# stardist/stardist

Hardware: AMD Instinct MI355X
Metric: predict_instances() Mpix/s (2D) + Mvox/s (3D) end-to-end at 1/2/4/8 GPU (higher is better)
Workload: dtype f32

## Files before the change

### include/stardist_hip.h

```cpp
#ifndef STARDIST_HIP_H
#define STARDIST_HIP_H

#include <stdbool.h>
#include <stdint.h>

#ifdef __cplusplus
extern "C" {
#endif

const char* sd_last_error(void);
int sd_version(void);
int sd_device_count(void);
int sd_release_workspace(void);
int sd_set_option(const char* name, int value);
int sd_get_option(const char* name);

int sd_nms2d_host(const float* dist, const float* points, int n_polys, int n_rays,
                  int use_kdtree, int use_bbox, int verbose, float threshold,
                  uint8_t* keep, int64_t* stats);
int sd_nms2d_device(const float* d_dist, const float* d_points, int n_polys, int n_rays,
                    int use_kdtree, int use_bbox, int verbose, float threshold,
                    uint8_t* d_keep, int64_t* stats, void* stream);

int sd_nms2d_old_host(const int32_t* polys, int n_polys, int n_rays, const int32_t* mapping, int height, int width,
                      float threshold, int max_bbox_search, int grid_y, int grid_x, int verbose, uint8_t* keep);
int sd_nms2d_old_device(const int32_t* d_polys, int n_polys, int n_rays, const int32_t* d_mapping, int height, int width,
                        float threshold, int max_bbox_search, int grid_y, int grid_x, int verbose, uint8_t* d_keep, void* stream);

int sd_prepare_polys_device(const int32_t* d_x, const int32_t* d_y, int n_polys, int n_verts, void* d_out,
                            int64_t out_bytes, void* stream);

int sd_clip_pairs_device(const int32_t* d_xa, const int32_t* d_ya, const int32_t* d_xb,
                         const int32_t* d_yb, int n_pairs, int n_verts,
                         int64_t* d_out_twice_area, int32_t* d_out_flags, void* stream);

int sd_area_bounds_pairs_device(const int32_t* d_xa, const int32_t* d_ya, const int32_t* d_xb, const int32_t* d_yb, int n_pairs,
                                int n_verts, float* d_out_area, float* d_out_band, int32_t* d_out_info, void* stream);

int sd_poly_pass_device(const int32_t* d_x, const int32_t* d_y, int n_polys, int n_verts, void* d_props, void* d_prep, void* stream);

int sd_star_dist2d_host(const uint16_t* src, int H, int W, int n_rays, int grid_y, int grid_x,
                        float* dst);
int sd_star_dist2d_device(const uint16_t* d_src, int H, int W, int n_rays, int grid_y,
                          int grid_x, float* d_dst, void* stream);
int sd_star_dist3d_host(const uint16_t* src, int Z, int Y, int X, const float* dz,
                        const float* dy, const float* dx, int n_rays, int grid_z, int grid_y,
                        int grid_x, float* dst);
int sd_star_dist3d_device(const uint16_t* d_src, int Z, int Y, int X, const float* d_dz,
                          const float* d_dy, const float* d_dx, int n_rays, int grid_z,
                          int grid_y, int grid_x, float* d_dst, void* stream);

int sd_edt_prob_device(const int32_t* d_lbl, int Z, int Y, int X, double sz, double sy, double sx, int max_label,
                       float* d_prob, void* stream);

int sd_polygons_to_label_host(const float* coord, const int32_t* labels, int n_polys, int n_rays,
                              int H, int W, int32_t* result);
int sd_polygons_to_label_device(const float* d_coord, const int32_t* d_labels, int n_polys,
                                int n_rays, int H, int W, int32_t* d_result, void* stream);
int sd_polygons_to_label_window_device(const float* d_coord, const int32_t* d_labels, int n_polys, int n_rays, int HI, int WI,
                                       int y0, int x0, int H, int W, int32_t* d_result, void* stream);

int sd_dist_to_coord_device(const float* d_dist, const double* d_points, const double* d_sincos, long long n_polys, int n_rays,
                            double scale_y, double scale_x, float* d_coord, void* stream);

int sd_survivor_positions_device(const unsigned char* d_keep, long long n, long long* d_positions, int32_t* d_count, void* stream);
int sd_survivors2d_device(const long long* d_positions, int m, const float* d_prob, const long long* d_points, const float* d_dist,
                          int n_rays, const double* d_sincos, float* d_out_prob, long long* d_out_points, float* d_out_coord,
                          float* d_out_coord_paint, int32_t* d_out_labels_paint, void* stream);

void _LIB_non_maximum_suppression_sparse(const float* scores, const float* dist,
                                         const float* points, const int n_polys,
                                         const int n_rays, const int n_faces, const float* verts,
                                         const int* faces, const float threshold,
                                         const int use_bbox, const int use_kdtree,
                                         const int verbose, bool* result);
int sd_nms3d_device(const float* d_scores, const float* d_dist, const float* d_points,
                    int n_polys, int n_rays, int n_faces, const float* d_verts,
                    const int* d_faces, float threshold, int use_bbox, int use_kdtree,
                    int verbose, uint8_t* d_keep, int64_t* stats, void* stream);

int sd_hiv_pairs_device(const float* d_dist, const float* d_points, int n_polys, int n_rays, int n_faces,
                        const float* d_verts, const int* d_faces, const int32_t* d_pairs, int n_pairs,
                        double* d_vol_kernel, double* d_vol_hull, void* stream);

void _LIB_polyhedron_to_label(const float* dist, const float* points, const float* verts,
                              const int* faces, const int n_polys, const int n_rays,
                              const int n_faces, const int* labels, const int nz, const int ny,
                              const int nx, const int render_mode, const int verbose,
                              const int use_overlap_label, const int overlap_label, int* result);
int sd_polyhedron_to_label_device(const float* d_dist, const float* d_points,
                                  const float* d_verts, const int* d_faces, int n_polys,
                                  int n_rays, int n_faces, const int* d_labels, int nz, int ny,
                                  int nx, int render_mode, int verbose, int use_overlap_label,
                                  int overlap_label, int* d_result, void* stream);
int sd_polyhedron_to_label_window_device(const float* d_dist, const float* d_points, const float* d_verts, const int* d_faces,
                                         int n_polys, int n_rays, int n_faces, const int* d_labels, int NZ, int NY, int NX,
                                         int z0, int y0, int x0, int nz, int ny, int nx, int render_mode, int verbose,
                                         int use_overlap_label, int overlap_label, int* d_result, void* stream);

int sd_select_candidates_device(const float* d_prob, const float* d_dist, int ndim,
                                const int* shape, const int* b, int n_rays, float thresh,
                                int cap, float* d_out_prob, float* d_out_dist,
                                int32_t* d_out_points, int32_t* d_count, void* stream);

int sd_sort_scores_desc_device(const float* d_scores, int n, float* d_sorted, int64_t* d_order, void* stream);

int sd_sorted_rows_device(const int32_t* d_points, const int64_t* d_order, int n, int ndim, const int* full_shape, const int* origin,
                          const int* grid, int64_t* d_rows, float* d_points_f32, int64_t* d_points_i64, void* stream);

void _LIB_non_maximum_suppression_2d(const float* dist, const float* points, const int n_polys,
                                     const int n_rays, const float threshold, const int use_bbox,
                                     const int use_kdtree, const int verbose, bool* result);
void _LIB_polygon_to_label(const float* coord, const int* labels, const int n_polys,
                           const int n_rays, const int ny, const int nx, int* result);
void _LIB_star_dist(const unsigned short* src, const int ny, const int nx, const int n_rays,
                    const int grid_y, const int grid_x, float* dst);
void _LIB_star_dist3d(const unsigned short* src, const int nz, const int ny, const int nx,
                      const float* pdz, const float* pdy, const float* pdx, const int n_rays,
                      const int grid_z, const int grid_y, const int grid_x, float* dst);

int sd_bias_act_device(float* d_x, const float* d_bias, long long n_outer, int n_channels,
                       long long inner, int act, void* stream);
int sd_add_bias_act_device(float* d_x, const float* d_addend, const float* d_bias, long long n_outer,
                           int n_channels, long long inner, int act, void* stream);

int sd_maxpool_ndhwc_device(const float* d_in, int n_channels, int D, int H, int W, int pz, int py, int px, float* d_out, void* stream);

int sd_inside_polyhedron_device(const float* d_dist, const float* d_centre, int n_rays, int n_faces,
                                const float* d_verts, const int* d_faces, const float* d_points,
                                long long n, int use_cone_map, uint8_t* d_out, void* stream);

int sd_bias_act_dot_device(const float* d_in, float* d_out, const float* d_bias, long long n_pix, int n_channels,
                           int act, const float* d_w, const float* d_wbias, int sigmoid, float* d_dot, void* stream);
int sd_head_rows_device(const float* d_feat, int n_channels, const long long* d_rows, long long n_rows,
                        const float* d_w, const float* d_bias, int n_out, float clamp_min, float* d_out,
                        void* stream);

long long sd_conv3_packed_floats(int c_in, int c_out, int kz);
int sd_conv3_pack_weights_host(const float* w , int c_in, int c_out, int kz, float* packed);
int sd_conv3_ndhwc_device(const float* d_src0, int c0, int stride0, int up0, const float* d_src1, int c1, int stride1, int up1,
                          int D, int H, int W, int kz, const float* d_wpacked, const float* d_bias, int c_out, int act,
                          float* d_out, void* stream);
int sd_conv3_res_ndhwc_device(const float* d_src0, int c0, int stride0, int up0, const float* d_src1, int c1, int stride1, int up1,
                              int D, int H, int W, int kz, const float* d_wpacked, const float* d_bias, const float* d_res,
                              int res_stride, int c_out, int act, float* d_out, void* stream);

long long sd_conv3_bf16x6_packed_floats(int c_in, int c_out, int kz);
int sd_conv3_bf16x6_pack_weights_host(const float* w , int c_in, int c_out, int kz, float* packed);
int sd_conv3_bf16x6_ndhwc_device(const float* d_src0, int c0, int stride0, int up0, const float* d_src1, int c1, int stride1,
                                 int up1, int D, int H, int W, int kz, const float* d_wpacked, const float* d_bias, int c_out,
                                 int act, float* d_out, void* stream);
int sd_conv3_bf16x6_res_ndhwc_device(const float* d_src0, int c0, int stride0, int up0, const float* d_src1, int c1, int stride1,
                                     int up1, int D, int H, int W, int kz, const float* d_wpacked, const float* d_bias,
                                     const float* d_res, int res_stride, int c_out, int act, float* d_out, void* stream);

long long sd_conv3_f16x3_packed_floats(int c_in, int c_out, int kz);
int sd_conv3_f16x3_pack_weights_host(const float* w , int c_in, int c_out, int kz, float* packed);
int sd_conv3_f16x3_ndhwc_device(const float* d_src0, int c0, int stride0, int up0, const float* d_src1, int c1, int stride1,
                                int up1, int D, int H, int W, int kz, const float* d_wpacked, const float* d_bias, int c_out,
                                int act, float* d_out, int* d_range_flag, void* stream);
int sd_conv3_f16x3_res_ndhwc_device(const float* d_src0, int c0, int stride0, int up0, const float* d_src1, int c1, int stride1,
                                    int up1, int D, int H, int W, int kz, const float* d_wpacked, const float* d_bias,
                                    const float* d_res, int res_stride, int c_out, int act, float* d_out, int* d_range_flag,
                                    void* stream);

int sd_conv3_f16x3_dot_ndhwc_device(const float* d_src0, int c0, int stride0, int up0, const float* d_src1, int c1, int stride1,
                                    int up1, int D, int H, int W, int kz, const float* d_wpacked, const float* d_bias, int c_out,
                                    int act, float* d_out, int* d_range_flag, const float* d_dot_w, float* d_dot_partial, void* stream);
int sd_dot_combine_device(const float* d_partial, int groups, long long n_pix, const float* d_wbias, int sigmoid, float* d_out, void* stream);

int sd_conv3_f16x3_fmt_ndhwc_device(const float* d_src0, int c0, int up0, const float* d_src1, int c1, int up1, int D, int H, int W, int kz,
                                    const float* d_wpacked, const float* d_bias, int c_out, int act, float* d_out, int in_split16,
                                    int out_split16, int* d_range_flag, const float* d_dot_w, float* d_dot_partial, void* stream);
int sd_conv3_f16x3_rows_device(const float* d_src, int c_in, int in_split16, int D, int H, int W, int kz, const float* d_wpacked,
                               const float* d_bias, int c_out, int act, const long long* d_rows, long long n_rows, float* d_out, void* stream);
int sd_conv3_c1x32_split16_device(const float* d_src, int D, int H, int W, int kz, const float* d_wpacked, const float* d_bias, int act,
                                  float* d_out, int* d_range_flag, void* stream);
int sd_maxpool_split16_ndhwc_device(const float* d_in, int n_channels, int D, int H, int W, int pz, int py, int px, float* d_out, void* stream);
int sd_split16_pack_device(const float* d_in, long long n_pix, int n_channels, float* d_out, int* d_range_flag, void* stream);
int sd_split16_unpack_device(const float* d_in, long long n_pix, int n_channels, float* d_out, void* stream);

int sd_upcat_ndhwc_device(const float* d_a, int ca, int up, const float* d_b, int cb, int D, int H, int W, float* d_out, void* stream);

long long sd_convg_packed_floats(int c_in, int c_out, int kz, int ky, int kx);
int sd_convg_pack_weights_host(const float* w , int c_in, int c_out, int kz, int ky, int kx, float* packed);
int sd_convg_ndhwc_device(const float* d_src, int c_in, int src_stride, int D, int H, int W, int kz, int ky, int kx, int sz, int sy,
                          int sx, int pz, int py, int px, int Do, int Ho, int Wo, const float* d_wpacked, const float* d_bias,
                          const float* d_res, int res_stride, int c_out, int act, float* d_out, int out_stride, void* stream);

int sd_label_overlap_device(const int32_t* d_true, const int32_t* d_pred, long long n, long long cap, int64_t* d_keys, int64_t* d_counts,
                            long long* h_count, int32_t* h_minmax, void* stream);

int sd_label_overlap_stack_device(const int32_t* d_ys, int K, long long n, long long cap, int64_t* d_keys, int64_t* d_counts,
                                  long long* h_offsets, long long* h_count, int32_t* h_minmax, void* stream);

int sd_relabel_stack_device(const int32_t* d_ys, int K, long long n, const int32_t* d_ids, const int32_t* d_new,
                            const long long* h_offsets, const int32_t* h_max, int32_t* d_out, void* stream);

int sd_conv_wgrad_ndhwc_device(const float* d_g, int c_out, const float* d_src0, int c0, int up0, const float* d_src1, int c1, int up1,
                               int B, int H, int W, int k, float* d_dw, float* d_db, void* stream);
int sd_relu_mask_device(const float* d_dy, const float* d_y, long long n, float* d_out, void* stream);
int sd_maxpool_adjoint_ndhwc_device(const float* d_in, const float* d_gout, int n_channels, int B, int H, int W, int py, int px,
                                    float* d_gin, void* stream);
int sd_upcat_adjoint_ndhwc_device(const float* d_gcat, int c0, int up0, int c1, int B, int H, int W, float* d_g0, float* d_g1, void* stream);
int sd_stardist_loss2d_device(const float* d_prob, const float* d_dist, const float* d_prob_true, const float* d_dist_true_mask,
                              long long n_pix, int n_rays, int dist_loss, double w_prob, double w_dist, double background_reg,
                              double* d_losses, float* d_grad_logit, float* d_grad_dist, void* stream);
int sd_stardist_loss2d_metrics_device(const float* d_prob, const float* d_dist, const float* d_prob_true, const float* d_dist_true_mask,
                                      long long n_pix, int n_rays, int dist_loss, double w_prob, double w_dist, double background_reg,
                                      double* d_losses, float* d_grad_logit, float* d_grad_dist, double* d_metrics, void* stream);

int sd_conv3_wgrad_ndhwc_device(const float* d_g, int c_out, const float* d_src0, int c0, int up0, const float* d_src1, int c1, int up1,
                                int B, int D, int H, int W, float* d_dw, float* d_db, void* stream);
int sd_convg_wgrad_ndhwc_device(const float* d_g, int c_out, const float* d_src, int c_in, int B, int D, int H, int W, int kz, int ky,
                                int kx, int sz, int sy, int sx, int pz, int py, int px, int Do, int Ho, int Wo, float* d_dw, float* d_db,
                                void* stream);
int sd_convg_dgrad_ndhwc_device(const float* d_g, int c_out, const float* d_wt, int c_in, int B, int D, int H, int W, int kz, int ky,
                                int kx, int sz, int sy, int sx, int pz, int py, int px, int Do, int Ho, int Wo, float* d_gin, void* stream);
int sd_maxpool3d_adjoint_ndhwc_device(const float* d_in, const float* d_gout, int n_channels, int B, int D, int H, int W, int pz, int py,
                                      int px, float* d_gin, void* stream);
int sd_upcat3d_adjoint_ndhwc_device(const float* d_gcat, int c0, int up0, int c1, int B, int D, int H, int W, float* d_g0, float* d_g1,
                                    void* stream);

int sd_class_targets_device(const int32_t* d_labels, int B, int D, int H, int W, const int32_t* d_meta, const int32_t* d_keys,
                            const int32_t* d_codes, const int32_t* d_tz, const int32_t* d_ty, const int32_t* d_tx, int d, int h, int w,
                            const unsigned char* d_neg, int n_channels, float* d_out, int32_t* d_missing, void* stream);
int sd_class_loss_device(const float* d_logits, const float* d_target, const double* d_class_weights, long long n_pix, int n_channels,
                         double w_class, double* d_losses, float* d_grad_logits, void* stream);

int sd_percentiles_device(const void* d_x, int dtype, long long n, int n_seg, const double* h_q, int n_q, int interp_f32, float* d_out,
                          void* stream);
int sd_normalize_mi_ma_device(const void* d_x, int dtype, long long n, int n_seg, const float* d_mi, const float* d_ma, float eps, int clip,
                              float* d_out, void* stream);

#ifdef __cplusplus
}
#endif
#endif
```

### stardist_amd/csrc/nms2d.hip

```cpp
#include <type_traits>

#include "common.h"
#include "clip_sweep.h"
#include "clip_beam.h"
#include "area_bounds.h"
#include "poly_pass.h"
#include "nms_rounds.h"
#include "../../include/stardist_hip.h"
#include <hipcub/hipcub.hpp>
#include <math.h>
#include <stdlib.h>
#include <vector>

namespace {

using sdclip::i64;

__device__ __forceinline__ float wave_min(float v) { for (int o = 32; o; o >>= 1) v = fminf(v, __shfl_xor(v, o)); return v; }
__device__ __forceinline__ float wave_max(float v) { for (int o = 32; o; o >>= 1) v = fmaxf(v, __shfl_xor(v, o)); return v; }
__device__ __forceinline__ i64 wave_sum(i64 v) { for (int o = 32; o; o >>= 1) v += __shfl_xor(v, o); return v; }

__global__ void __launch_bounds__(256) k_build(const float* __restrict__ dist, const float* __restrict__ pts,
                                               const float2* __restrict__ sincos, int N, int R,
                                               int* __restrict__ vx, int* __restrict__ vy, int4* __restrict__ bbox,
                                               float* __restrict__ radius, float* __restrict__ area, int* gstats) {
  extern __shared__ int lds[];
  const int wave = threadIdx.x >> 6, lane = threadIdx.x & 63;
  const int i = blockIdx.x * (blockDim.x >> 6) + wave;
  if (i >= N) return;
  int* sx = lds + wave * 2 * R;
  int* sy = sx + R;
  const float py = pts[2 * i], px = pts[2 * i + 1];
  float xmin = INFINITY, xmax = -INFINITY, ymin = INFINITY, ymax = -INFINITY, rmax = 0.f;
  for (int k = lane; k < R; k += 64) {
    const float d = dist[(size_t)i * R + k];
    const float2 sc = sincos[k];
    const float y = py + d * sc.x;
    const float x = px + d * sc.y;
    xmin = fminf(xmin, x); xmax = fmaxf(xmax, x);
    ymin = fminf(ymin, y); ymax = fmaxf(ymax, y);
    const int X = (int)(long long)x, Y = (int)(long long)y;
    sx[k] = X; sy[k] = Y;
    vx[(size_t)i * R + k] = X; vy[(size_t)i * R + k] = Y;
    rmax = fmaxf(rmax, d);
  }
  xmin = wave_min(xmin); xmax = wave_max(xmax); ymin = wave_min(ymin); ymax = wave_max(ymax);
  rmax = wave_max(rmax);
  __builtin_amdgcn_wave_barrier();
  i64 s = 0, sa = 0;
  for (int k = lane; k < R; k += 64) {
    const int kn = (k + 1 == R) ? 0 : k + 1;
    const i64 c = (i64)sx[k] * sy[kn] - (i64)sy[k] * sx[kn];
    s += c; sa += (c < 0 ? -c : c);
  }
  s = wave_sum(s); sa = wave_sum(sa);
  if (lane == 0) {
    float a;
    if (sa < (1ll << 24)) a = (float)s;
    else {
      a = 0.f;
      for (int k = 0; k < R; ++k) {
        const int kn = (k + 1 == R) ? 0 : k + 1;
        a += (float)((i64)sx[k] * sy[kn] - (i64)sy[k] * sx[kn]);
      }
    }
    area[i] = (float)(0.5 * (double)fabsf(a));
    radius[i] = rmax;
    bbox[i] = make_int4((int)xmin, (int)xmax, (int)ymin, (int)ymax);
    const int rb = __float_as_int(rmax);
    const int iy = (int)floorf(py), ix = (int)floorf(px);
    volatile int* gs = gstats;
    if (rb > gs[0]) atomicMax(&gstats[0], rb);
    if (iy < gs[1]) atomicMin(&gstats[1], iy);
    if (iy > gs[2]) atomicMax(&gstats[2], iy);
    if (ix < gs[3]) atomicMin(&gstats[3], ix);
    if (ix > gs[4]) atomicMax(&gstats[4], ix);
  }
}

__global__ void __launch_bounds__(256) k_build32(const float* __restrict__ dist, const float* __restrict__ pts,
                                                 const float2* __restrict__ sincos, int N, int R,
                                                 int* __restrict__ vx, int* __restrict__ vy, int4* __restrict__ bbox,
                                                 float* __restrict__ radius, float* __restrict__ area, int* gstats) {
  __shared__ int sxy[8][2][32];
  const int l = threadIdx.x & 31, hw = threadIdx.x >> 5;
  const int i = blockIdx.x * 8 + hw;
  const bool cv = i < N, lv = cv && l < R;
  int* sx = sxy[hw][0];
  int* sy = sxy[hw][1];
  float py = 0.f, px = 0.f;
  if (cv) { py = pts[2 * i]; px = pts[2 * i + 1]; }
  float xmin = INFINITY, xmax = -INFINITY, ymin = INFINITY, ymax = -INFINITY, rmax = 0.f;
  if (lv) {
    const float d = dist[(size_t)i * R + l];
    const float2 sc = sincos[l];
    const float y = py + d * sc.x;
    const float x = px + d * sc.y;
    xmin = xmax = x; ymin = ymax = y;
    const int X = (int)(long long)x, Y = (int)(long long)y;
    sx[l] = X; sy[l] = Y;
    vx[(size_t)i * R + l] = X; vy[(size_t)i * R + l] = Y;
    rmax = fmaxf(0.f, d);
  }
  for (int o = 16; o; o >>= 1) {
    xmin = fminf(xmin, __shfl_xor(xmin, o)); xmax = fmaxf(xmax, __shfl_xor(xmax, o));
    ymin = fminf(ymin, __shfl_xor(ymin, o)); ymax = fmaxf(ymax, __shfl_xor(ymax, o));
    rmax = fmaxf(rmax, __shfl_xor(rmax, o));
  }
  __builtin_amdgcn_wave_barrier();
  i64 s = 0, sa = 0;
  if (lv) {
    const int kn = (l + 1 == R) ? 0 : l + 1;
    const i64 c = (i64)sx[l] * sy[kn] - (i64)sy[l] * sx[kn];
    s = c; sa = (c < 0 ? -c : c);
  }
  for (int o = 16; o; o >>= 1) { s += __shfl_xor(s, o); sa += __shfl_xor(sa, o); }
  if (cv && l == 0) {
    float a;
    if (sa < (1ll << 24)) a = (float)s;
    else {
      a = 0.f;
      for (int k = 0; k < R; ++k) {
        const int kn = (k + 1 == R) ? 0 : k + 1;
        a += (float)((i64)sx[k] * sy[kn] - (i64)sy[k] * sx[kn]);
      }
    }
    area[i] = (float)(0.5 * (double)fabsf(a));
    radius[i] = rmax;
    bbox[i] = make_int4((int)xmin, (int)xmax, (int)ymin, (int)ymax);
    const int rb = __float_as_int(rmax);
    const int iy = (int)floorf(py), ix = (int)floorf(px);
    volatile int* gs = gstats;
    if (rb > gs[0]) atomicMax(&gstats[0], rb);
    if (iy < gs[1]) atomicMin(&gstats[1], iy);
    if (iy > gs[2]) atomicMax(&gstats[2], iy);
    if (ix < gs[3]) atomicMin(&gstats[3], ix);
    if (ix > gs[4]) atomicMax(&gstats[4], ix);
  }
}

struct GridP { float y0, x0, inv_cs; int ny, nx; };

__device__ __forceinline__ int cell_of(const GridP g, float py, float px, int& cy, int& cx) {
  cy = (int)((py - g.y0) * g.inv_cs); cx = (int)((px - g.x0) * g.inv_cs);
  cy = min(max(cy, 0), g.ny - 1); cx = min(max(cx, 0), g.nx - 1);
  return cy * g.nx + cx;
}

struct Window { int ylo, yhi, xlo, xhi; };
__device__ __forceinline__ Window cell_window(const GridP g, bool by_bbox, float reach, const int4 bb, float py, float px) {
  float y0, y1, x0, x1;
  if (by_bbox) { x0 = (float)bb.x - reach; x1 = (float)bb.y + reach; y0 = (float)bb.z - reach; y1 = (float)bb.w + reach; }
  else { const float rr = 2.f * reach; x0 = px - rr; x1 = px + rr; y0 = py - rr; y1 = py + rr; }
  Window w;
  w.ylo = min(max((int)floorf((y0 - 0.5f - g.y0) * g.inv_cs), 0), g.ny - 1); w.yhi = min(max((int)floorf((y1 + 0.5f - g.y0) * g.inv_cs), 0), g.ny - 1);
  w.xlo = min(max((int)floorf((x0 - 0.5f - g.x0) * g.inv_cs), 0), g.nx - 1); w.xhi = min(max((int)floorf((x1 + 0.5f - g.x0) * g.inv_cs), 0), g.nx - 1);
  return w;
}
constexpr int MAX_WIN_ROWS = 32;

__global__ void k_cell_count(const float* __restrict__ pts, int N, GridP g, int* __restrict__ cellCount, int* __restrict__ candCell) {
  const int i = blockIdx.x * blockDim.x + threadIdx.x;
  if (i >= N) return;
  int cy, cx;
  const int c = cell_of(g, pts[2 * i], pts[2 * i + 1], cy, cx);
  candCell[i] = c;
  atomicAdd(&cellCount[c], 1);
}
struct __attribute__((aligned(16))) CellRec { int4 bb; float py, px, area; int j; };
__global__ void k_cell_fill(int N, const int* __restrict__ candCell, const int* __restrict__ cellStart,
                            int* __restrict__ cellFill, const float* __restrict__ pts, const int4* __restrict__ bbox,
                            const float* __restrict__ area, CellRec* __restrict__ rec, GridP g, int by_bbox, float reach, int* __restrict__ slotCap) {
  const int i = blockIdx.x * blockDim.x + threadIdx.x;
  if (i >= N) return;
  const int c = candCell[i];
  const int pos = atomicAdd(&cellFill[c], 1);
  CellRec r;
  r.bb = bbox[i]; r.py = pts[2 * i]; r.px = pts[2 * i + 1]; r.area = area[i]; r.j = i;
  rec[cellStart[c] + pos] = r;
  if (slotCap) {
    const Window w = cell_window(g, by_bbox != 0, reach, r.bb, r.py, r.px);
    int u = -1;
    for (int yy = w.ylo; yy <= w.yhi; ++yy) u += cellStart[yy * g.nx + w.xhi + 1] - cellStart[yy * g.nx + w.xlo];
    slotCap[i] = u;
  }
}

__device__ __forceinline__ bool bbox_intersect(const int4 a, const int4 b) {
  return (b.x <= a.y && a.x <= b.y && b.z <= a.w && a.z <= b.w);
}

__device__ __forceinline__ bool may_interact(const NmsFlags f, const int4 bi, const int4 bj, float pyi, float pxi, float pyj, float pxj,
                                             float ai, float aj) {
  if (f.thr_nonneg) {
    if (!bbox_intersect(bi, bj)) return false;
    const float wh = (float)(min(bi.y, bj.y) - max(bi.x, bj.x)) * (float)(min(bi.w, bj.w) - max(bi.z, bj.z));
    return wh * 1.00001f >= f.thr * fminf(ai, aj) * 0.99999f;
  }
  bool ok = true;
  if (f.use_bbox) ok = ok && bbox_intersect(bi, bj);
  if (f.use_kdtree) {
    const float dy = pyi - pyj, dxx = pxi - pxj;
    const float rr = 2.f * f.max_dist + 1.f;
    ok = ok && (dy * dy + dxx * dxx < rr * rr);
  }
  return ok;
}

template <int MODE>
__global__ void __launch_bounds__(256) k_neighbours(int N, GridP g, NmsFlags f, const CellRec* __restrict__ rec, const int* __restrict__ cellStart,
                                                    int* __restrict__ nbrCount, int* __restrict__ nbrLow, const i64* __restrict__ nbrStart,
                                                    int* __restrict__ nbr, int* __restrict__ waitOn, int by_bbox, float reach, unsigned long long* __restrict__ total) {
  const int wave = threadIdx.x >> 6, lane = threadIdx.x & 63;
  const int per = gridDim.x >> 3;
  const int blk = (blockIdx.x & 7) * per + (blockIdx.x >> 3);
  const int w = blk * (blockDim.x >> 6) + wave;
  if (w >= N) return;
  const CellRec me = rec[w];
  const int i = me.j;
  int cy, cx;
  cell_of(g, me.py, me.px, cy, cx);
  const int4 bi = me.bb;
  const float pyi = me.py, pxi = me.px, ai = me.area;
  int nLo = 0, nHi = 0;
  int minj = INT32_MAX;
  const i64 baseLo = MODE ? nbrStart[i] : 0;
  const i64 baseHi = MODE == 1 ? baseLo + nbrLow[i] : (MODE == 2 ? nbrStart[i + 1] - 1 : 0);
  const Window win = cell_window(g, by_bbox != 0, reach, bi, pyi, pxi);
  const int nrows = win.yhi - win.ylo + 1;
  int rbeg = 0, rlen = 0;
  if (lane < nrows) { rbeg = cellStart[(win.ylo + lane) * g.nx + win.xlo]; rlen = cellStart[(win.ylo + lane) * g.nx + win.xhi + 1] - rbeg; }
  int incl = rlen;
  for (int o = 1; o < MAX_WIN_ROWS; o <<= 1) { const int t = __shfl_up(incl, o); if (lane >= o) incl += t; }
  const int total_recs = __shfl(incl, nrows - 1);
  const int excl = incl - rlen;
  for (int t = 0; t < total_recs; t += 64) {
    const int v = t + lane;
    bool hit = false;
    int j = -1;
    {
      int rb = 0, re = 0;
      for (int r = 0; r < nrows; ++r) {
        const int e_r = __shfl(excl, r), b_r = __shfl(rbeg, r);
        if (e_r <= v) { rb = b_r; re = e_r; }
      }
      if (v < total_recs) {
        const CellRec r = rec[rb + (v - re)];
        j = r.j;
        if (j != i) hit = may_interact(f, bi, r.bb, pyi, pxi, r.py, r.px, ai, r.area);
      }
    }
    const unsigned long long mLo = __ballot(hit && j < i), mHi = __ballot(hit && j > i);
    if (MODE && hit) {
      const unsigned long long below = (1ull << lane) - 1;
      if (j < i) { nbr[baseLo + nLo + __popcll(mLo & below)] = j; if (j < minj) minj = j; }
      else if (MODE == 1) nbr[baseHi + nHi + __popcll(mHi & below)] = j;
      else nbr[baseHi - (nHi + __popcll(mHi & below))] = j;
    }
    nLo += __popcll(mLo); nHi += __popcll(mHi);
  }
  if (!MODE && lane == 0) { nbrCount[i] = nLo + nHi; nbrLow[i] = nLo; }
  if (MODE == 2 && lane == 0) nbrLow[i] = nLo;
  if (MODE && lane == 0) nbrCount[i] = nHi;
  if (MODE) {
    for (int o = 32; o; o >>= 1) minj = min(minj, __shfl_xor(minj, o));
    if (lane == 0) waitOn[i] = (minj < i) ? minj : WAIT_NONE;
  }
}

constexpr int EMIT_STAGE = 512;
__global__ void __launch_bounds__(256) k_round_emit(const int* __restrict__ K, const int* __restrict__ nKPtr, unsigned char* __restrict__ state,
                                                    const i64* __restrict__ nbrStart, const int* __restrict__ nbrHigh, const int* __restrict__ nbr, NmsFlags f,
                                                    const float* __restrict__ pts, const int4* __restrict__ bbox,
                                                    const float* __restrict__ radius, const float* __restrict__ area,
                                                    int2* __restrict__ pairs, unsigned long long* pairCount,
                                                    unsigned long long pairCap) {
  const int wave = threadIdx.x >> 6, lane = threadIdx.x & 63;
  const int nK = *nKPtr;
  __shared__ int2 stage[4][EMIT_STAGE];
  int nst = 0;
  auto flush = [&]() {
    if (!nst) return;
    unsigned long long base = 0;
    if (lane == 0) base = atomicAdd(pairCount, (unsigned long long)nst);
    base = __shfl(base, 0);
    __builtin_amdgcn_wave_barrier();
    for (int k = lane; k < nst; k += 64) { const unsigned long long pos = base + k; if (pos < pairCap) pairs[pos] = stage[wave][k]; }
    __builtin_amdgcn_wave_barrier();
    nst = 0;
  };
  for (int w = blockIdx.x * (blockDim.x >> 6) + wave; w < nK; w += gridDim.x * (blockDim.x >> 6)) {
  const int i = K[w];
  if (lane == 0) state[i] = ST_KEPT;
  const i64 end = nbrStart[i + 1], beg = end - nbrHigh[i];
  const int4 bi = bbox[i];
  const float pyi = pts[2 * i], pxi = pts[2 * i + 1];
  const float rad = f.max_dist + radius[i];
  const float rad2 = rad * rad;
  for (i64 t = beg; t < end; t += 64) {
    const i64 idx = t + lane;
    bool emit = false;
    int j = -1;
    if (idx < end) {
      j = nbr[idx];
      if (j > i && state[j] == ST_UNDECIDED) {
        bool ok = true;
        if (f.use_kdtree) {
          const float d0 = pyi - pts[2 * j], d1 = pxi - pts[2 * j + 1];
          float d2 = d0 * d0; d2 += d1 * d1;
          ok = d2 < rad2;
        }
        if (ok && (f.use_bbox || f.thr_nonneg)) {
          const int4 bj = bbox[j];
          ok = bbox_intersect(bi, bj);
          if (ok && f.thr_nonneg) {
            const double w = (double)(min(bi.y, bj.y) - max(bi.x, bj.x)), hgt = (double)(min(bi.w, bj.w) - max(bi.z, bj.z));
            const float ub = (float)((w * hgt) / fmin((double)area[i] + 1.e-10, (double)area[j] + 1.e-10));
            if (!(ub > f.thr)) ok = false;
          }
        }
        emit = ok;
      }
    }
    const unsigned long long m = __ballot(emit);
    if (m) {
      const int c = __popcll(m);
      if (nst + c > EMIT_STAGE) flush();
      if (emit) stage[wave][nst + __popcll(m & ((1ull << lane) - 1))] = make_int2(i, j);
      nst += c;
    }
  }
  }
  flush();
}

template <int MAXV, int S>
__global__ void __launch_bounds__(S) k_prepare(const int* __restrict__ vx, const int* __restrict__ vy, int N, int R,
                                               sdclip::PolyPrep<MAXV>* __restrict__ prep) {
  const int i = blockIdx.x * S + threadIdx.x;
  if (i >= N) return;
  sdclip::PrepWork<sdclip::LdsStorage<S>, MAXV> w;
  w.prepare(vx + (size_t)i * R, vy + (size_t)i * R, R, prep + i);
}

struct PairQueues { unsigned int* spill; unsigned int* spillCount; unsigned int* exact; unsigned int* exactCount; unsigned int cap; };
enum { BEAM_CAPFLAGS = sdclip::ST_OVERFLOW_IL | sdclip::ST_OVERFLOW_REC | sdclip::ST_OVERFLOW_AEL | sdclip::ST_OVERFLOW_LM | sdclip::ST_OVERFLOW_GJ };
template <int MAXV, int K, int MAXIL, int MAXREC, int S, typename CNT, bool REL16 = false>
__global__ void __launch_bounds__(S) k_pairs_beam(const int2* __restrict__ pairs, const unsigned int* __restrict__ idx, const CNT* __restrict__ nPtr,
                                                  const unsigned int* __restrict__ firstPtr, const sdclip::PolyPrep<MAXV>* __restrict__ prep,
                                                  const float* __restrict__ area, float thr, unsigned char* __restrict__ state,
                                                  unsigned char* __restrict__ supp, PairQueues q) {
  typedef typename std::conditional<REL16, sdclip::LdsStorage16<S>, sdclip::LdsStorage<S>>::type Storage;
  typedef sdclip::Beam<MAXV, K, MAXIL, MAXREC, Storage> BeamT;
  const unsigned long long n = (unsigned long long)*nPtr;
  const unsigned long long first = firstPtr ? (unsigned long long)*firstPtr : 0ull;
  const unsigned long long total = n > first ? n - first : 0ull;
  const unsigned long long chunk = (total + gridDim.x - 1) / gridDim.x;
  const bool spread = chunk <= (unsigned long long)S;
  unsigned long long t = spread ? first + (unsigned long long)blockIdx.x * chunk + threadIdx.x : first + (unsigned long long)blockIdx.x * S + threadIdx.x;
  if (spread && (unsigned long long)threadIdx.x >= chunk) t = n;
  const unsigned long long step = spread ? (1ull << 62) : (unsigned long long)gridDim.x * S;
  for (; t < n; t += step) {
    const unsigned int p = idx ? idx[t] : (unsigned int)t;
    const int2 ij = pairs[p];
    BeamT bm;
    bm.reset_state(prep + ij.x, prep + ij.y);
    const i64 twice = bm.execute();
    const int st = bm.status;
    if (st & BEAM_CAPFLAGS) {
      const unsigned int k = atomicAdd(q.spillCount, 1u);
      if (k < q.cap) q.spill[k] = p;
      continue;
    }
    if ((st & ~sdclip::ST_FAIL) || bm.n_joins > 0 || bm.sum_abs_terms >= (1ll << 24)) {
      const unsigned int k = atomicAdd(q.exactCount, 1u);
      if (k < q.cap) q.exact[k] = p;
      continue;
    }
    const float area_inter = 0.5f * (float)twice;
    const float overlap = (float)((double)area_inter / fmin((double)area[ij.x] + 1.e-10, (double)area[ij.y] + 1.e-10));
    if (overlap > thr) { if (supp) supp[p] = 1; else state[ij.y] = ST_SUPPRESSED; }
  }
}
template <int MAXV, int K, int MAXIL, int MAXREC, int S, bool REL16 = false>
size_t beam_lds_bytes() {
  typedef typename std::conditional<REL16, sdclip::LdsStorage16<S>, sdclip::LdsStorage<S>>::type Storage;
  return (size_t)sdclip::Beam<MAXV, K, MAXIL, MAXREC, Storage>::lds_bytes() + 64;
}

__global__ void __launch_bounds__(256) k_pairs_decide(const int2* __restrict__ pairs, const unsigned long long* __restrict__ nPtr,
                                                      const unsigned int* __restrict__ firstPtr, const int* __restrict__ vx, const int* __restrict__ vy, int R,
                                                      const sdarea::PolyProps* __restrict__ props, const float* __restrict__ area, float thr,
                                                      unsigned char* __restrict__ state, unsigned char* __restrict__ supp,
                                                      unsigned char* __restrict__ decided, unsigned int* __restrict__ nDecided) {
  __shared__ float2 sq[4][2][32];
  const int lane = threadIdx.x & 63, half = lane >> 5, l = lane & 31, wv = threadIdx.x >> 6;
  const unsigned long long n = *nPtr, first = firstPtr ? (unsigned long long)*firstPtr : 0ull;
  const unsigned long long nw = (unsigned long long)gridDim.x * 4;
  unsigned int mine = 0;
  for (unsigned long long base = first + 2ull * ((unsigned long long)blockIdx.x * 4 + wv); base < n; base += 2ull * nw) {
    const unsigned long long t = base + half;
    const bool active = t < n;
    const int2 ij = active ? pairs[t] : make_int2(0, 0);
    const sdarea::PolyProps pp = props[ij.x], pq = props[ij.y];
    const sdarea::Enclosure E = sdarea::pair_enclosure(vx + (size_t)ij.x * R, vy + (size_t)ij.x * R, vx + (size_t)ij.y * R, vy + (size_t)ij.y * R, R, pp, pq,
                                                       active, sq[wv][half], l, half);
    if (active && l == 0) {
      const int dec = sdarea::decide(E, area[ij.x], area[ij.y], thr);
      decided[t] = (unsigned char)dec;
      if (dec == 2) { if (supp) supp[t] = 1; else state[ij.y] = ST_SUPPRESSED; }
      if (dec) ++mine;
    }
    __builtin_amdgcn_wave_barrier();
  }
  mine += __shfl_xor(mine, 32);
  if (lane == 0 && mine) atomicAdd(nDecided, mine);
}

__global__ void __launch_bounds__(256) k_tail_emit(const int* __restrict__ U, int nU, const unsigned char* __restrict__ state,
                                                   const i64* __restrict__ nbrStart, const int* __restrict__ nbrLow, const int* __restrict__ nbr, NmsFlags f,
                                                   const float* __restrict__ pts, const int4* __restrict__ bbox,
                                                   const float* __restrict__ radius, const float* __restrict__ area,
                                                   int2* __restrict__ pairs, unsigned long long* pairCount, unsigned long long pairCap,
                                                   unsigned int* __restrict__ segStart, int* __restrict__ segCnt) {
  const int wave = threadIdx.x >> 6, lane = threadIdx.x & 63;
  for (int w = blockIdx.x * (blockDim.x >> 6) + wave; w < nU; w += gridDim.x * (blockDim.x >> 6)) {
    const int j = U[w];
    int cnt = 0;
    unsigned long long base = 0;
    if (state[j] == ST_UNDECIDED) {
      const i64 beg = nbrStart[j], end = beg + nbrLow[j];
      const int4 bj = bbox[j];
      const float pyj = pts[2 * j], pxj = pts[2 * j + 1];
      const float aj = area[j];
      for (int pass = 0; pass < 2; ++pass) {
        int k = 0;
        for (i64 t = beg; t < end; t += 64) {
          const i64 id = t + lane;
          bool emit = false;
          int i = -1;
          if (id < end) {
            i = nbr[id];
            if (i < j && state[i] == ST_UNDECIDED) {
              bool ok = true;
              if (f.use_kdtree) {
                const float rad = f.max_dist + radius[i];
                const float d0 = pts[2 * i] - pyj, d1 = pts[2 * i + 1] - pxj;
                float d2 = d0 * d0; d2 += d1 * d1;
                ok = d2 < rad * rad;
              }
              if (ok && (f.use_bbox || f.thr_nonneg)) {
                const int4 bi = bbox[i];
                ok = bbox_intersect(bi, bj);
                if (ok && f.thr_nonneg) {
                  const double w2 = (double)(min(bi.y, bj.y) - max(bi.x, bj.x)), hgt = (double)(min(bi.w, bj.w) - max(bi.z, bj.z));
                  const float ub = (float)((w2 * hgt) / fmin((double)area[i] + 1.e-10, (double)aj + 1.e-10));
                  if (!(ub > f.thr)) ok = false;
                }
              }
              emit = ok;
            }
          }
          const unsigned long long m = __ballot(emit);
          if (pass == 1 && emit) {
            const unsigned long long pos = base + k + __popcll(m & ((1ull << lane) - 1));
            if (pos < pairCap) pairs[pos] = make_int2(i, j);
          }
          k += __popcll(m);
        }
        if (pass == 0) {
          cnt = k;
          if (cnt == 0) break;
          if (lane == 0) base = atomicAdd(pairCount, (unsigned long long)cnt);
          base = __shfl(base, 0);
        }
      }
    }
    if (lane == 0) { segStart[w] = (unsigned int)base; segCnt[w] = cnt; }
  }
}
struct Deferred { int2* pairs; int* next; int* head; unsigned char* pend; unsigned int* count; unsigned int cap; };
__global__ void k_defer(const int2* __restrict__ pairs, const unsigned int* __restrict__ exact, const unsigned int* __restrict__ nExact, unsigned int qcap,
                        Deferred d, unsigned int* __restrict__ nErr) {
  unsigned int n = *nExact; if (n > qcap) n = qcap;
  for (unsigned int t = blockIdx.x * blockDim.x + threadIdx.x; t < n; t += gridDim.x * blockDim.x) {
    const int2 ij = pairs[exact[t]];
    const unsigned int k = atomicAdd(d.count, 1u);
    if (k < d.cap) { d.pairs[k] = ij; d.pend[ij.y] = 1; d.next[k] = atomicExch(&d.head[ij.y], (int)k); }
    else atomicAdd(nErr, 1u);
  }
}
__global__ void k_tail_init(Deferred d, int2* __restrict__ pairs, unsigned int* __restrict__ exact, unsigned long long* nPairs,
                            unsigned int* nExact, unsigned int* firstNew) {
  unsigned int n = *d.count; if (n > d.cap) n = d.cap;
  for (unsigned int t = blockIdx.x * blockDim.x + threadIdx.x; t < n; t += gridDim.x * blockDim.x) { pairs[t] = d.pairs[t]; exact[t] = t; }
  if (blockIdx.x == 0 && threadIdx.x == 0) { *nPairs = n; *nExact = n; *firstNew = n; }
}
__global__ void k_defer_undecided(const int2* __restrict__ pairs, const unsigned long long* __restrict__ nPtr, const unsigned int* __restrict__ nDecided,
                                  unsigned int limit, unsigned char* __restrict__ decided, const unsigned char* __restrict__ state, Deferred d,
                                  unsigned char* __restrict__ kind, unsigned int* __restrict__ nErr) {
  const unsigned long long n = *nPtr;
  if (n - (unsigned long long)*nDecided > (unsigned long long)limit) return;
  for (unsigned long long t = (unsigned long long)blockIdx.x * blockDim.x + threadIdx.x; t < n; t += (unsigned long long)gridDim.x * blockDim.x) {
    if (decided[t]) continue;
    decided[t] = 4;
    const int2 ij = pairs[t];
    if (state[ij.y] == ST_SUPPRESSED) continue;
    const unsigned int k = atomicAdd(d.count, 1u);
    if (k < d.cap) { d.pairs[k] = ij; d.pend[ij.y] = 1; d.next[k] = atomicExch(&d.head[ij.y], (int)k); kind[k] = 1; }
    else atomicAdd(nErr, 1u);
  }
}
__global__ void k_tail_init2(Deferred d, const unsigned char* __restrict__ kind, int2* __restrict__ pairs, unsigned int* __restrict__ exact,
                             unsigned long long* nPairs, unsigned int* nExact, unsigned int* firstNew, unsigned char* __restrict__ decided) {
  unsigned int n = *d.count; if (n > d.cap) n = d.cap;
  for (unsigned int t = blockIdx.x * blockDim.x + threadIdx.x; t < n; t += gridDim.x * blockDim.x) {
    pairs[t] = d.pairs[t];
    if (kind[t] == 0) { exact[atomicAdd(nExact, 1u)] = t; decided[t] = 3; } else decided[t] = 0;
  }
  if (blockIdx.x == 0 && threadIdx.x == 0) { *nPairs = n; *firstNew = n; }
}
__global__ void k_copy_u32(unsigned int* dst, const unsigned int* src) { *dst = *src; }
__device__ __forceinline__ bool deferred_suppresses(int j, const int* __restrict__ defHead, const int* __restrict__ defNext,
                                                    const unsigned char* __restrict__ supp) {
  for (int k = defHead[j]; k >= 0; k = defNext[k]) if (supp[k]) return true;
  return false;
}

__global__ void __launch_bounds__(256) k_tail_step(const int* __restrict__ U, int nU, unsigned char* state, const int2* __restrict__ pairs,
                                                   const unsigned char* __restrict__ supp, const unsigned int* __restrict__ segStart,
                                                   const int* __restrict__ segCnt, unsigned long long pairCap,
                                                   const int* __restrict__ defHead, const int* __restrict__ defNext) {
  const int t = blockIdx.x * blockDim.x + threadIdx.x;
  if (t >= nU) return;
  const int j = U[t];
  if (state[j] != ST_UNDECIDED) return;
  bool wait = false, sup = deferred_suppresses(j, defHead, defNext, supp);
  const unsigned int e0 = segStart[t];
  const int c = segCnt[t];
  for (int e = 0; e < c && !sup; ++e) {
    if ((unsigned long long)e0 + e >= pairCap) { wait = true; break; }
    const unsigned char si = state[pairs[e0 + e].x];
    if (si == ST_UNDECIDED) wait = true;
    else if (si == ST_KEPT && supp[e0 + e]) sup = true;
  }
  if (sup) state[j] = ST_SUPPRESSED;
  else if (!wait) state[j] = ST_KEPT;
}
__global__ void __launch_bounds__(1024) k_tail_resolve(const int* __restrict__ U, int nU, volatile unsigned char* state,
                                                       const int2* __restrict__ pairs, const unsigned char* __restrict__ supp,
                                                       const unsigned int* __restrict__ segStart, const int* __restrict__ segCnt,
                                                       unsigned long long pairCap, int* left, const int* __restrict__ defHead,
                                                       const int* __restrict__ defNext) {
  __shared__ int changed, undecided;
  for (int iter = 0; iter <= nU; ++iter) {
    if (threadIdx.x == 0) { changed = 0; undecided = 0; }
    __syncthreads();
    for (int t = threadIdx.x; t < nU; t += blockDim.x) {
      const int j = U[t];
      if (state[j] != ST_UNDECIDED) continue;
      bool wait = false, sup = deferred_suppresses(j, defHead, defNext, supp);
      const unsigned int e0 = segStart[t];
      const int c = segCnt[t];
      for (int e = 0; e < c && !sup; ++e) {
        if ((unsigned long long)e0 + e >= pairCap) { wait = true; break; }
        const unsigned char si = state[pairs[e0 + e].x];
        if (si == ST_UNDECIDED) wait = true;
        else if (si == ST_KEPT && supp[e0 + e]) sup = true;
      }
      if (sup) { state[j] = ST_SUPPRESSED; changed = 1; }
      else if (!wait) { state[j] = ST_KEPT; changed = 1; }
      else undecided = 1;
    }
    __threadfence_block();
    __syncthreads();
    const int ch = changed, un = undecided;
    __syncthreads();
    if (!un || !ch) { if (threadIdx.x == 0) *left = un; break; }
  }
}

constexpr int PAIR_BUCKETS = 4096;
struct PairKey { const char* prep; size_t prepStride; float inv; int nl, ny, nx; };
__device__ __forceinline__ int pair_bucket(const float* __restrict__ pts, int2 ij, const PairKey& k) {
  const float dy = pts[2 * ij.y] - pts[2 * ij.x], dx = pts[2 * ij.y + 1] - pts[2 * ij.x + 1];
  int by = (int)((dy * k.inv + 0.5f) * (float)k.ny), bx = (int)((dx * k.inv + 0.5f) * (float)k.nx);
  by = by < 0 ? 0 : (by >= k.ny ? k.ny - 1 : by); bx = bx < 0 ? 0 : (bx >= k.nx ? k.nx - 1 : bx);
  int lm = 0;
  if (k.nl > 1) {
    int a = *(const int*)(k.prep + (size_t)ij.x * k.prepStride + 4), b = *(const int*)(k.prep + (size_t)ij.y * k.prepStride + 4);
    a = a < 1 ? 0 : (a > 4 ? 3 : a - 1); b = b < 1 ? 0 : (b > 4 ? 3 : b - 1);
    lm = (a * 4 + b) % k.nl;
  }
  return (lm * k.ny + by) * k.nx + bx;
}
__global__ void __launch_bounds__(256) k_pair_bucket_count(const int2* __restrict__ pairs, const unsigned long long* __restrict__ nPtr,
                                                           const unsigned int* __restrict__ firstPtr, const float* __restrict__ pts, PairKey key,
                                                           unsigned int* __restrict__ hist, const unsigned char* __restrict__ decided) {
  __shared__ unsigned int h[PAIR_BUCKETS];
  for (int b = threadIdx.x; b < PAIR_BUCKETS; b += 256) h[b] = 0;
  __syncthreads();
  const unsigned long long n = *nPtr, first = firstPtr ? *firstPtr : 0u;
  for (unsigned long long t = first + (unsigned long long)blockIdx.x * 256 + threadIdx.x; t < n; t += (unsigned long long)gridDim.x * 256)
    if (!decided || !decided[t]) atomicAdd(&h[pair_bucket(pts, pairs[t], key)], 1u);
  __syncthreads();
  for (int b = threadIdx.x; b < PAIR_BUCKETS; b += 256) if (h[b]) atomicAdd(&hist[b], h[b]);
}
__global__ void __launch_bounds__(1024) k_pair_bucket_scan(const unsigned int* __restrict__ hist, unsigned int* __restrict__ cursor,
                                                           unsigned long long* __restrict__ nOrdered) {
  __shared__ unsigned int sh[1024];
  const int t = threadIdx.x;
  unsigned int v[PAIR_BUCKETS / 1024], tot = 0;
#pragma unroll
  for (int k = 0; k < PAIR_BUCKETS / 1024; ++k) { v[k] = hist[t * (PAIR_BUCKETS / 1024) + k]; tot += v[k]; }
  sh[t] = tot;
  __syncthreads();
  for (int o = 1; o < 1024; o <<= 1) {
    const unsigned int add = t >= o ? sh[t - o] : 0u;
    __syncthreads();
    sh[t] += add;
    __syncthreads();
  }
  unsigned int run = sh[t] - tot;
#pragma unroll
  for (int k = 0; k < PAIR_BUCKETS / 1024; ++k) { cursor[t * (PAIR_BUCKETS / 1024) + k] = run; run += v[k]; }
  if (t == 1023) *nOrdered = sh[t];
}
__global__ void __launch_bounds__(256) k_pair_bucket_scatter(const int2* __restrict__ pairs, const unsigned long long* __restrict__ nPtr,
                                                             const unsigned int* __restrict__ firstPtr, const float* __restrict__ pts, PairKey key,
                                                             unsigned int* __restrict__ cursor, unsigned int* __restrict__ order, unsigned int cap,
                                                             const unsigned char* __restrict__ decided) {
  const unsigned long long n = *nPtr, first = firstPtr ? *firstPtr : 0u;
  for (unsigned long long t = first + (unsigned long long)blockIdx.x * 256 + threadIdx.x; t < n; t += (unsigned long long)gridDim.x * 256) {
    if (decided && decided[t]) continue;
    const unsigned int k = atomicAdd(&cursor[pair_bucket(pts, pairs[t], key)], 1u);
    if (k < cap) order[k] = (unsigned int)t;
  }
}

__global__ void k_count_after(unsigned int* out, const unsigned int* total, const unsigned int* first) { *out = *total > *first ? *total - *first : 0u; }

}

namespace sd {
int clip_full_pairs(const int2* d_pairs, const unsigned int* d_idx, const unsigned int* d_n, unsigned int cap, int R, const int* d_vx, const int* d_vy,
                    const float* d_area, float thr, unsigned char* d_state, unsigned char* d_supp, unsigned int* d_errCount, hipStream_t stream);
}

namespace {
struct Counters { int nU, nK, nS, left; unsigned long long nPairs; unsigned int nSpill, nExact, nErr, nDecided; };

template <int MAXV, int SPREP>
struct BeamPath {
  typedef sdclip::PolyPrep<MAXV> Prep;
  static int prepare(const int* vx, const int* vy, int N, int R, void* prep, hipStream_t s) {
    if constexpr (MAXV == 32) {
      if (sdpass::launch_poly_pass(vx, vy, N, R, nullptr, prep, s)) { sd::set_error("sd_nms2d: launch of the per-polygon pass failed"); return -1; }
      return 0;
    } else {
      const size_t lds = sdclip::PrepWork<sdclip::LdsStorage<SPREP>, MAXV>::lds_bytes() + 64;
      hipLaunchKernelGGL((k_prepare<MAXV, SPREP>), dim3(sd::div_up(N, SPREP)), dim3(SPREP), lds, s, vx, vy, N, R, (Prep*)prep);
      SD_LAUNCH_CHECK();
      return 0;
    }
  }
  static int tier1(const int2* pairs, const unsigned int* idx, const unsigned long long* nPairs, const unsigned int* first, const void* prep, const float* area,
                   float thr, unsigned char* state, unsigned char* supp, PairQueues q, hipStream_t s) {
    const int lanes = sd::option(sd::OPT_NMS2D_PAIR_LANES);
    if (lanes == 32) {
      static const size_t lds32 = beam_lds_bytes<MAXV, 8, 6, 4, 32>();
      hipLaunchKernelGGL((k_pairs_beam<MAXV, 8, 6, 4, 32, unsigned long long>), dim3(256 * 8), dim3(32), lds32, s, pairs, idx, nPairs, first, (const Prep*)prep, area, thr, state, supp, q);
    } else if (lanes == 6464) {
      static const size_t lds = beam_lds_bytes<MAXV, 8, 6, 4, 64>();
      hipLaunchKernelGGL((k_pairs_beam<MAXV, 8, 6, 4, 64, unsigned long long>), dim3(256 * 4), dim3(64), lds, s, pairs, idx, nPairs, first, (const Prep*)prep, area, thr, state, supp, q);
    } else {
      static const size_t lds16 = beam_lds_bytes<MAXV, 8, 6, 4, 64, true>();
      static const int per_cu = (int)((160 * 1024) / lds16);
      hipLaunchKernelGGL((k_pairs_beam<MAXV, 8, 6, 4, 64, unsigned long long, true>), dim3(256 * per_cu), dim3(64), lds16, s, pairs, idx, nPairs, first, (const Prep*)prep, area, thr, state, supp, q);
    }
    SD_LAUNCH_CHECK();
    return 0;
  }
  template <typename CNT>
  static int tier2(const int2* pairs, const unsigned int* idx, const CNT* nPairs, const unsigned int* first, const void* prep, const float* area, float thr,
                   unsigned char* state, unsigned char* supp, PairQueues q, hipStream_t s) {
    static const size_t lds = beam_lds_bytes<MAXV, 15, 16, 8, 32>();
    hipLaunchKernelGGL((k_pairs_beam<MAXV, 15, 16, 8, 32, CNT>), dim3(256 * 3), dim3(32), lds, s, pairs, idx, nPairs, first, (const Prep*)prep, area, thr, state, supp, q);
    SD_LAUNCH_CHECK();
    return 0;
  }
};
}

extern "C" int sd_nms2d_device(const float* d_dist, const float* d_points, int n_polys, int n_rays, int use_kdtree,
                               int use_bbox, int verbose, float threshold, uint8_t* d_keep, int64_t* stats,
                               void* stream_) {
  hipStream_t s = (hipStream_t)stream_;
  const int N = n_polys, R = n_rays;
  if (stats) memset(stats, 0, 16 * sizeof(int64_t));
  if (N <= 0) return 0;
  if (R < 1 || R > 256) { sd::set_error("sd_nms2d: n_rays=%d unsupported (1..256)", R); return -1; }
  if (verbose) {
    printf("Non Maximum Suppression (2D) ++++ \n");
    printf("NMS: n_polys    = %d \nNMS: n_rays     = %d  \nNMS: thresh     = %.3f \nNMS: use_bbox   = %d\nNMS: use_kdtree = %d\n",
           N, R, threshold, use_bbox, use_kdtree);
    printf("NMS: using HIP (gfx950), uniform-grid broad phase + scan-beam pair kernel\n");
  }
  sd::Arena& A = sd::arena();
  if (A.begin(s)) return -1;
  hipEvent_t ev0 = nullptr, ev1 = nullptr;
  if (stats) { SD_CHECK(hipEventCreate(&ev0)); SD_CHECK(hipEventCreate(&ev1)); }
  struct EvGuard { hipEvent_t a, b; ~EvGuard() { if (a) (void)hipEventDestroy(a); if (b) (void)hipEventDestroy(b); } } evguard{ev0, ev1};
  double ns_pairs = 0, ns_full = 0, ns_pre = 0;
  long long n_pair_launches = 0;

  if (!use_kdtree && !use_bbox && threshold < 0) {
    SD_CHECK(hipMemsetAsync(d_keep, 0, N, s));
    SD_CHECK(hipMemsetAsync(d_keep, 1, 1, s));
    SD_CHECK(hipStreamSynchronize(s));
    return 0;
  }

  std::vector<float2> sc(R);
  const float ANGLE_PI = 2 * M_PI / R;
  for (int k = 0; k < R; ++k) { sc[k].x = sinf(ANGLE_PI * k); sc[k].y = cosf(ANGLE_PI * k); }
  float2* d_sc = A.take_n<float2>(R);
  int* vx = A.take_n<int>((size_t)N * R);
  int* vy = A.take_n<int>((size_t)N * R);
  int4* bbox = A.take_n<int4>(N);
  float* radius = A.take_n<float>(N);
  float* area = A.take_n<float>(N);
  int* gstats = A.take_n<int>(8);
  unsigned char* state = A.take_n<unsigned char>(N);
  int* candCell = A.take_n<int>(N);
  if (!d_sc || !vx || !vy || !bbox || !radius || !area || !gstats || !state || !candCell) return -1;
  SD_CHECK(hipMemcpyAsync(d_sc, sc.data(), R * sizeof(float2), hipMemcpyHostToDevice, s));
  const int gs_init[8] = {0, INT32_MAX, INT32_MIN, INT32_MAX, INT32_MIN, 0, 0, 0};
  SD_CHECK(hipMemcpyAsync(gstats, gs_init, sizeof(gs_init), hipMemcpyHostToDevice, s));
  SD_CHECK(hipMemsetAsync(state, 0, N, s));
  if (stats) SD_CHECK(hipEventRecord(ev0, s));
  if (R <= 32)
    hipLaunchKernelGGL(k_build32, dim3(sd::div_up(N, 8)), dim3(256), 0, s, d_dist, d_points, d_sc, N, R, vx, vy, bbox, radius, area, gstats);
  else
    hipLaunchKernelGGL(k_build, dim3(sd::div_up(N, 4)), dim3(256), 4 * 2 * R * sizeof(int), s, d_dist, d_points, d_sc, N, R,
                       vx, vy, bbox, radius, area, gstats);
  SD_LAUNCH_CHECK();
  size_t prepStride;
  if (R <= 32) prepStride = sizeof(sdclip::PolyPrep<32>); else if (R <= 64) prepStride = sizeof(sdclip::PolyPrep<64>);
  else if (R <= 128) prepStride = sizeof(sdclip::PolyPrep<128>); else prepStride = sizeof(sdclip::PolyPrep<256>);
  void* prep = A.take((size_t)N * prepStride);
  if (!prep) return -1;
  hipStream_t side = sd::side_stream();
  if (!side) return -1;
  hipEvent_t evFork = nullptr, evJoin = nullptr;
  SD_CHECK(hipEventCreateWithFlags(&evFork, hipEventDisableTiming));
  SD_CHECK(hipEventCreateWithFlags(&evJoin, hipEventDisableTiming));
  EvGuard evguardFJ{evFork, evJoin};
  const bool areaBounds = R <= 32 && R >= 3 && sd::option(sd::OPT_NMS2D_AREA_BOUNDS) != 0 && sd::option(sd::OPT_NMS2D_STRICT) == 0;
  sdarea::PolyProps* props = nullptr;
  hipEvent_t evProps = nullptr, evPrep = nullptr;
  SD_CHECK(hipEventCreateWithFlags(&evProps, hipEventDisableTiming));
  SD_CHECK(hipEventCreateWithFlags(&evPrep, hipEventDisableTiming));
  EvGuard evguardP{evProps, evPrep};
  if (areaBounds) {
    props = (sdarea::PolyProps*)A.take((size_t)N * sizeof(sdarea::PolyProps));
    if (!props) return -1;
  }
  auto launch_side = [&]() -> int {
    SD_CHECK(hipEventRecord(evFork, s));
    SD_CHECK(hipStreamWaitEvent(side, evFork, 0));
    int rc;
    if (R <= 32) rc = sdpass::launch_poly_pass(vx, vy, N, R, props, prep, side);
    else if (R <= 64) rc = BeamPath<64, 64>::prepare(vx, vy, N, R, prep, side);
    else if (R <= 128) rc = BeamPath<128, 32>::prepare(vx, vy, N, R, prep, side);
    else rc = BeamPath<256, 16>::prepare(vx, vy, N, R, prep, side);
    if (rc) { sd::set_error("sd_nms2d: launch of the per-polygon pass failed"); return -1; }
    SD_CHECK(hipEventRecord(evProps, side));
    SD_CHECK(hipEventRecord(evPrep, side));
    SD_CHECK(hipEventRecord(evJoin, side));
    return 0;
  };
  int gs[8];
  SD_CHECK(hipMemcpyAsync(gs, gstats, sizeof(gs), hipMemcpyDeviceToHost, s));
  SD_CHECK(hipStreamSynchronize(s));
  float max_dist;
  memcpy(&max_dist, &gs[0], 4);

  GridP g;
  const float reach = (max_dist + 1.f) * 1.0001f + 1e-3f;
  const int by_bbox = (threshold >= 0.f || use_bbox) ? 1 : 0;
  float cs = 0.5f * reach;
  if (!(cs >= 1.f)) cs = 1.f;
  for (;;) {
    g.ny = (int)(((double)gs[2] - gs[1]) / cs) + 1;
    g.nx = (int)(((double)gs[4] - gs[3]) / cs) + 1;
    if ((long long)g.ny * g.nx <= (1ll << 26)) break;
    cs *= 2.f;
  }
  g.y0 = (float)gs[1]; g.x0 = (float)gs[3]; g.inv_cs = 1.f / cs;
  const int nCells = g.ny * g.nx;
  int* cellCount = A.take_n<int>(nCells + 1);
  int* cellStart = A.take_n<int>(nCells + 1);
  int* cellFill = A.take_n<int>(nCells + 1);
  CellRec* cellRec = (CellRec*)A.take((size_t)N * sizeof(CellRec));
  int* nbrCount = A.take_n<int>(N + 1);
  i64* nbrStart = A.take_n<i64>(N + 1);
  int* nbrLow = A.take_n<int>(N + 1);
  if (!cellCount || !cellStart || !cellFill || !cellRec || !nbrCount || !nbrStart || !nbrLow) return -1;
  SD_CHECK(hipMemsetAsync(cellCount, 0, (nCells + 1) * sizeof(int), s));
  SD_CHECK(hipMemsetAsync(cellFill, 0, (nCells + 1) * sizeof(int), s));
  hipLaunchKernelGGL(k_cell_count, dim3(sd::div_up(N, 256)), dim3(256), 0, s, d_points, N, g, cellCount, candCell);
  SD_LAUNCH_CHECK();
  size_t tmpBytes = 0, tmpBytes2 = 0;
  (void)hipcub::DeviceScan::ExclusiveSum(nullptr, tmpBytes, cellCount, cellStart, nCells + 1, s);
  (void)hipcub::DeviceScan::ExclusiveSum(nullptr, tmpBytes2, nbrCount, nbrStart, N + 1, s);
  if (tmpBytes2 > tmpBytes) tmpBytes = tmpBytes2;
  void* scanTmp = A.take(tmpBytes + 256);
  if (!scanTmp) return -1;
  SD_CHECK(hipcub::DeviceScan::ExclusiveSum(scanTmp, tmpBytes, cellCount, cellStart, nCells + 1, s));
  const bool singlePass = sd::option(sd::OPT_NMS2D_NBR_SINGLE) != 0;
  SD_CHECK(hipMemsetAsync(nbrCount, 0, (N + 1) * sizeof(int), s));
  hipLaunchKernelGGL(k_cell_fill, dim3(sd::div_up(N, 256)), dim3(256), 0, s, N, candCell, cellStart, cellFill, d_points, bbox, area, cellRec, g, by_bbox, reach,
                     singlePass ? nbrCount : (int*)nullptr);
  SD_LAUNCH_CHECK();
  int* U0 = A.take_n<int>(N);
  unsigned char* pend0 = A.take_n<unsigned char>(N);
  int* head0 = A.take_n<int>(N);
  unsigned int* dcount0 = A.take_n<unsigned int>(1);
  if (!U0 || !pend0 || !head0 || !dcount0) return -1;
  hipLaunchKernelGGL(k_iota, dim3(sd::div_up(N, 256)), dim3(256), 0, s, U0, N);
  SD_CHECK(hipMemsetAsync(pend0, 0, N, s));
  SD_CHECK(hipMemsetAsync(head0, 0xFF, (size_t)N * sizeof(int), s));
  SD_CHECK(hipMemsetAsync(dcount0, 0, sizeof(unsigned int), s));

  NmsFlags f;
  f.use_kdtree = use_kdtree; f.use_bbox = use_bbox; f.thr_nonneg = (threshold >= 0.f); f.thr = threshold; f.max_dist = max_dist;

  const int nbBlocks = (sd::div_up(N, 4) + 7) & ~7;
  NbrLists L{};
  L.count = nbrCount; L.low = nbrLow; L.start = nbrStart;
  auto launch_neighbours = [&](int mode, const NbrLists& l) {
    if (mode == 0)
      hipLaunchKernelGGL((k_neighbours<0>), dim3(nbBlocks), dim3(256), 0, s, N, g, f, cellRec, cellStart, nbrCount, nbrLow, (const i64*)nullptr, (int*)nullptr,
                         (int*)nullptr, by_bbox, reach, (unsigned long long*)nullptr);
    else if (mode == 1)
      hipLaunchKernelGGL((k_neighbours<1>), dim3(nbBlocks), dim3(256), 0, s, N, g, f, cellRec, cellStart, nbrCount, nbrLow, (const i64*)nbrStart, l.nbr, l.waitOn, by_bbox, reach,
                         (unsigned long long*)nullptr);
    else
      hipLaunchKernelGGL((k_neighbours<2>), dim3(nbBlocks), dim3(256), 0, s, N, g, f, cellRec, cellStart, nbrCount, nbrLow, (const i64*)nbrStart, l.nbr, l.waitOn, by_bbox, reach,
                         (unsigned long long*)nullptr);
  };
  const int rcLists = build_neighbour_lists(A, s, N, singlePass, scanTmp, tmpBytes, launch_neighbours, launch_side, L);
  if (rcLists > 0) {
    sd::set_error("sd_nms2d: %lld neighbour entries for %d candidates exceed the capacity of one call (2^31 - 1): shard the input "
                  "(predict_instances_sharded / predict_instances_big)", (long long)L.total, N);
    return -1;
  }
  if (rcLists) return -1;
  const int* nbr = L.nbr;
  int* waitOn = L.waitOn;
  const i64 totalNbr = L.total;

  SD_CHECK(hipStreamWaitEvent(s, evProps, 0));
  if (stats) { SD_CHECK(hipEventRecord(ev1, s)); SD_CHECK(hipEventSynchronize(ev1)); float ms = 0; SD_CHECK(hipEventElapsedTime(&ms, ev0, ev1)); ns_pre = ms * 1e6; }

  const unsigned long long pairCap = (unsigned long long)(totalNbr / 2 + 64);
  int* U1 = A.take_n<int>(N);
  int* K = A.take_n<int>(N);
  int2* pairs = A.take_n<int2>(pairCap);
  const unsigned int qCap = (unsigned int)(pairCap < (1ull << 30) ? pairCap : (1ull << 30));
  unsigned int* spillPairs = A.take_n<unsigned int>(qCap);
  unsigned int* exactPairs = A.take_n<unsigned int>(qCap);
  int* Sl = A.take_n<int>(N);
  Counters* d_cnt = (Counters*)A.take(sizeof(Counters));
  static const bool pairSort = sd::tuning_env("SD_NMS_PAIR_SORT", 1) != 0;
  unsigned int* pairOrder = pairSort && R <= 32 ? A.take_n<unsigned int>(qCap) : nullptr;
  unsigned int* bucketHist = A.take_n<unsigned int>(2 * PAIR_BUCKETS);
  unsigned long long* nOrdered = A.take_n<unsigned long long>(1);
  if (!U0 || !U1 || !K || !pairs || !spillPairs || !exactPairs || !Sl || !d_cnt || !bucketHist || !nOrdered || (pairSort && R <= 32 && !pairOrder)) return -1;
  unsigned char* decided = (areaBounds && pairOrder) ? A.take_n<unsigned char>(pairCap) : nullptr;
  if (areaBounds && pairOrder && !decided) return -1;
  i64 totalDecided = 0;
  int nU = N, rounds = 0;
  i64 totalPairs = 0, totalExact = 0, totalSpill = 0;
  int* Ucur = U0; int* Unext = U1;
  Counters h;
  hipEvent_t ev2 = nullptr, ev3 = nullptr;
  if (stats) { SD_CHECK(hipEventCreate(&ev2)); SD_CHECK(hipEventCreate(&ev3)); }
  EvGuard evguard2{ev2, ev3};
  static const int tailDiv = sd::tuning_env("SD_NMS_TAIL_DIV", 6);
  static const int tailMax = sd::tuning_env("SD_NMS_TAIL_MAX", 65536);
  const int tailT = tailDiv > 0 ? ((N / tailDiv) < tailMax ? (N / tailDiv) : tailMax) : -1;
  unsigned char* supp = nullptr; unsigned int* segStart = nullptr; int* segCnt = nullptr;
  static const bool deferEnv = sd::tuning_env("SD_NMS_DEFER", 1) != 0;
  const bool deferOn = tailT >= 0 && deferEnv;
  Deferred dfr{nullptr, nullptr, nullptr, nullptr, nullptr, qCap};
  unsigned int* firstNew = A.take_n<unsigned int>(1);
  dfr.pend = pend0; dfr.head = head0; dfr.count = dcount0;
  if (!firstNew) return -1;
  if (deferOn) {
    dfr.pairs = A.take_n<int2>(qCap);
    dfr.next = A.take_n<int>(qCap);
    if (!dfr.pairs || !dfr.next) return -1;
  }
  i64 nDeferred = 0;
  bool sideGeneral = false;
  unsigned int* nNewExact = A.take_n<unsigned int>(1);
  if (!nNewExact) return -1;
  const int deferFrom = (deferOn && decided) ? sd::option(sd::OPT_NMS2D_DEFER_UNDECIDED) : 0;
  const unsigned int deferMax = (unsigned int)(sd::option(sd::OPT_NMS2D_DEFER_MAX) > 0 ? sd::option(sd::OPT_NMS2D_DEFER_MAX) : 0);
  unsigned char* defKind = nullptr; unsigned int* nJoinDef = nullptr;
  if (deferFrom > 0) {
    defKind = A.take_n<unsigned char>(qCap); nJoinDef = A.take_n<unsigned int>(1);
    if (!defKind || !nJoinDef) return -1;
    SD_CHECK(hipMemsetAsync(defKind, 0, qCap, s));
  }
  i64 totalUndecDeferred = 0;
  i64 nUndecDeferredUpper = 0;
  auto run_pairs = [&](unsigned char* suppOut) -> int {
    const unsigned int* first = suppOut ? firstNew : nullptr;
    if (stats) SD_CHECK(hipEventRecord(ev0, s));
    PairQueues q1{spillPairs, &d_cnt->nSpill, exactPairs, &d_cnt->nExact, qCap};
    PairQueues q2{exactPairs, &d_cnt->nExact, exactPairs, &d_cnt->nExact, qCap};
    int rc;
    if (R <= 32) {
      if (pairOrder) {
        static const int keyMode = sd::tuning_env("SD_NMS_PAIR_KEY", 2);
        static const int modes[6][3] = {{1, 32, 32}, {1, 64, 16}, {1, 64, 64}, {16, 16, 16}, {16, 32, 8}, {4, 32, 32}};
        const int* md = modes[keyMode >= 0 && keyMode < 6 ? keyMode : 2];
        const PairKey key{(const char*)prep, prepStride, 1.f / (4.f * (max_dist + 1.f)), md[0], md[1], md[2]};
        SD_CHECK(hipMemsetAsync(bucketHist, 0, PAIR_BUCKETS * sizeof(unsigned int), s));
        if (decided)
          hipLaunchKernelGGL(k_pairs_decide, dim3(256 * 8), dim3(256), 0, s, pairs, &d_cnt->nPairs, first, vx, vy, R, props, area, threshold, state, suppOut,
                             decided, &d_cnt->nDecided);
        if (!suppOut && deferFrom > 0 && rounds >= deferFrom)
          hipLaunchKernelGGL(k_defer_undecided, dim3(256), dim3(256), 0, s, pairs, &d_cnt->nPairs, &d_cnt->nDecided, deferMax, decided, state, dfr, defKind, &d_cnt->nErr);
        const unsigned int* bfirst = (suppOut && deferFrom > 0) ? nullptr : first;
        SD_CHECK(hipStreamWaitEvent(s, evPrep, 0));
        hipLaunchKernelGGL(k_pair_bucket_count, dim3(512), dim3(256), 0, s, pairs, &d_cnt->nPairs, bfirst, d_points, key, bucketHist, decided);
        hipLaunchKernelGGL(k_pair_bucket_scan, dim3(1), dim3(1024), 0, s, bucketHist, bucketHist + PAIR_BUCKETS, nOrdered);
        hipLaunchKernelGGL(k_pair_bucket_scatter, dim3(512), dim3(256), 0, s, pairs, &d_cnt->nPairs, bfirst, d_points, key, bucketHist + PAIR_BUCKETS,
                           pairOrder, qCap, decided);
        SD_LAUNCH_CHECK();
        rc = BeamPath<32, 64>::tier1(pairs, pairOrder, nOrdered, (const unsigned int*)nullptr, prep, area, threshold, state, suppOut, q1, s);
      } else {
        SD_CHECK(hipStreamWaitEvent(s, evPrep, 0));
        rc = BeamPath<32, 64>::tier1(pairs, (const unsigned int*)nullptr, &d_cnt->nPairs, first, prep, area, threshold, state, suppOut, q1, s);
      }
      if (stats) SD_CHECK(hipEventRecord(ev1, s));
      if (!rc) rc = BeamPath<32, 64>::tier2(pairs, spillPairs, &d_cnt->nSpill, (const unsigned int*)nullptr, prep, area, threshold, state, suppOut, q2, s);
    } else {
      SD_CHECK(hipStreamWaitEvent(s, evPrep, 0));
      if (R <= 64) rc = BeamPath<64, 64>::tier2(pairs, (const unsigned int*)nullptr, &d_cnt->nPairs, first, prep, area, threshold, state, suppOut, q2, s);
      else if (R <= 128) rc = BeamPath<128, 32>::tier2(pairs, (const unsigned int*)nullptr, &d_cnt->nPairs, first, prep, area, threshold, state, suppOut, q2, s);
      else rc = BeamPath<256, 16>::tier2(pairs, (const unsigned int*)nullptr, &d_cnt->nPairs, first, prep, area, threshold, state, suppOut, q2, s);
      if (stats) SD_CHECK(hipEventRecord(ev1, s));
    }
    if (rc) return -1;
    if (stats) SD_CHECK(hipEventRecord(ev2, s));
    if (!suppOut && deferOn) {
      hipLaunchKernelGGL(k_defer, dim3(64), dim3(256), 0, s, pairs, exactPairs, &d_cnt->nExact, qCap, dfr, &d_cnt->nErr);
      SD_LAUNCH_CHECK();
    } else if (suppOut && sideGeneral) {
      hipLaunchKernelGGL(k_count_after, dim3(1), dim3(1), 0, s, nNewExact, &d_cnt->nExact, deferFrom > 0 ? nJoinDef : firstNew);
      SD_LAUNCH_CHECK();
      if (sd::clip_full_pairs(pairs, exactPairs + nDeferred, nNewExact, qCap - (unsigned int)nDeferred, R, vx, vy, area, threshold, state, suppOut, &d_cnt->nErr, s)) return -1;
      SD_CHECK(hipStreamWaitEvent(s, evJoin, 0));
    } else if (sd::clip_full_pairs(pairs, exactPairs, &d_cnt->nExact, qCap, R, vx, vy, area, threshold, state, suppOut, &d_cnt->nErr, s)) return -1;
    if (stats) SD_CHECK(hipEventRecord(ev3, s));
    return 0;
  };
  auto account = [&](const char* what) -> int {
    if (h.nPairs > pairCap || h.nSpill > qCap || h.nExact > qCap) { sd::set_error("sd_nms2d: pair queue overflow (internal error)"); return -1; }
    if (h.nErr) { sd::set_error("sd_nms2d: %u pairs exceeded the general path's fixed capacities or the deferred-pair list (with more than 64 rays: at least that many; the launch stops at the first)", h.nErr); return -1; }
    totalPairs += (i64)h.nPairs; totalExact += h.nExact; totalSpill += h.nSpill; totalDecided += h.nDecided;
    if (stats) {
      float ms = 0, ms2 = 0;
      SD_CHECK(hipEventElapsedTime(&ms, ev0, ev1)); SD_CHECK(hipEventElapsedTime(&ms2, ev2, ev3));
      if (h.nPairs) { ns_pairs += ms * 1e6; ++n_pair_launches; }
      ns_full += ms2 * 1e6;
      if (sd::option(sd::OPT_TRACE)) printf("%s %d: nU=%d nK=%d pairs=%llu decided by the area enclosure=%u spill=%u exact=%u pair_kernel=%.3f ms general_path=%.3f ms\n", what, rounds, h.nU, h.nK, h.nPairs, h.nDecided, h.nSpill, h.nExact, ms, ms2);
    }
    return 0;
  };
  bool forceTail = false;
  while (nU > 0) {
    ++rounds;
    if (tailT >= 0 && ((nU <= tailT && rounds > 1) || forceTail)) {
      if (!supp) { supp = A.take_n<unsigned char>(pairCap); segStart = A.take_n<unsigned int>(N); segCnt = A.take_n<int>(N); }
      if (!supp || !segStart || !segCnt) return -1;
      SD_CHECK(hipMemsetAsync(d_cnt, 0, sizeof(Counters), s));
      SD_CHECK(hipMemsetAsync(supp, 0, pairCap, s));
      const int wg = sd::div_up(nU, 4) < 2048 ? sd::div_up(nU, 4) : 2048;
      if (deferFrom > 0) {
        hipLaunchKernelGGL(k_tail_init2, dim3(64), dim3(256), 0, s, dfr, defKind, pairs, exactPairs, &d_cnt->nPairs, &d_cnt->nExact, firstNew, decided);
        hipLaunchKernelGGL(k_copy_u32, dim3(1), dim3(1), 0, s, nJoinDef, &d_cnt->nExact);
      } else
        hipLaunchKernelGGL(k_tail_init, dim3(64), dim3(256), 0, s, dfr, pairs, exactPairs, &d_cnt->nPairs, &d_cnt->nExact, firstNew);
      sideGeneral = deferOn && nDeferred > 0 && nDeferred < (i64)qCap && side != nullptr;
      if (sideGeneral) {
        SD_CHECK(hipEventRecord(evFork, s));
        SD_CHECK(hipStreamWaitEvent(side, evFork, 0));
        if (sd::clip_full_pairs(pairs, exactPairs, deferFrom > 0 ? nJoinDef : firstNew, qCap, R, vx, vy, area, threshold, state, supp, &d_cnt->nErr, side)) return -1;
        SD_CHECK(hipEventRecord(evJoin, side));
      }
      hipLaunchKernelGGL(k_tail_emit, dim3(wg), dim3(256), 0, s, Ucur, nU, state, nbrStart, nbrLow, nbr, f, d_points, bbox, radius, area, pairs,
                         &d_cnt->nPairs, pairCap, segStart, segCnt);
      SD_LAUNCH_CHECK();
      if (run_pairs(supp)) return -1;
      hipEvent_t evr0 = nullptr, evr1 = nullptr;
      const bool tr = stats && sd::option(sd::OPT_TRACE);
      if (tr) { SD_CHECK(hipEventCreate(&evr0)); SD_CHECK(hipEventCreate(&evr1)); SD_CHECK(hipEventRecord(evr0, s)); }
      for (int it = 0; it < 10; ++it)
        hipLaunchKernelGGL(k_tail_step, dim3(sd::div_up(nU, 256)), dim3(256), 0, s, Ucur, nU, state, pairs, supp, segStart, segCnt, pairCap, dfr.head, dfr.next);
      hipLaunchKernelGGL(k_tail_resolve, dim3(1), dim3(1024), 0, s, Ucur, nU, state, pairs, supp, segStart, segCnt, pairCap, &d_cnt->left, dfr.head, dfr.next);
      SD_LAUNCH_CHECK();
      if (tr) { SD_CHECK(hipEventRecord(evr1, s)); SD_CHECK(hipEventSynchronize(evr1)); float ms = 0; SD_CHECK(hipEventElapsedTime(&ms, evr0, evr1));
                printf("tail replay (10 steps + resolve loop): %.3f ms\n", ms); (void)hipEventDestroy(evr0); (void)hipEventDestroy(evr1); }
      unsigned int hDefTotal = (unsigned int)nDeferred;
      SD_CHECK(hipMemcpyAsync(&h, d_cnt, sizeof(Counters), hipMemcpyDeviceToHost, s));
      if (deferFrom > 0) SD_CHECK(hipMemcpyAsync(&hDefTotal, dfr.count, sizeof(unsigned int), hipMemcpyDeviceToHost, s));
      SD_CHECK(hipStreamSynchronize(s));
      h.nU = nU; h.nK = 0;
      if (deferFrom > 0) { totalUndecDeferred = (i64)hDefTotal - nDeferred; if ((unsigned long long)hDefTotal <= h.nPairs) h.nPairs -= hDefTotal; }
      else
      if ((i64)h.nPairs >= nDeferred) h.nPairs -= (unsigned long long)nDeferred;
      if ((i64)h.nExact >= nDeferred) h.nExact -= (unsigned int)nDeferred;
      if (account("tail batch after round")) return -1;
      if (h.left) { sd::set_error("sd_nms2d: tail batch left candidates undecided (internal error)"); return -1; }
      nU = 0;
      break;
    }
    SD_CHECK(hipMemsetAsync(d_cnt, 0, sizeof(Counters), s));
    hipLaunchKernelGGL(k_round_triage, dim3(sd::div_up(nU, 1024)), dim3(1024), 0, s, Ucur, nU, state, waitOn, Unext, K, Sl, (int*)d_cnt, dfr.pend);
    const int wgrid = sd::div_up(nU, 4) < 2048 ? sd::div_up(nU, 4) : 2048;
    hipLaunchKernelGGL(k_round_scan, dim3(wgrid), dim3(256), 0, s, Sl, state, nbrStart, nbrLow, nbr, waitOn, Unext, K, (int*)d_cnt, dfr.pend);
    hipLaunchKernelGGL(k_round_emit, dim3(wgrid), dim3(256), 0, s, K, &d_cnt->nK, state, nbrStart, nbrCount, nbr, f, d_points, bbox,
                       radius, area, pairs, &d_cnt->nPairs, pairCap);
    SD_LAUNCH_CHECK();
    if (run_pairs(nullptr)) return -1;
    SD_CHECK(hipMemcpyAsync(&h, d_cnt, sizeof(Counters), hipMemcpyDeviceToHost, s));
    SD_CHECK(hipStreamSynchronize(s));
    if (h.nK == 0 && h.nU > 0) {
      if (deferOn && (nDeferred > 0 || nUndecDeferredUpper > 0) && !forceTail) forceTail = true;
      else { sd::set_error("sd_nms2d: greedy scan made no progress (internal error)"); return -1; }
    }
    if (deferOn) nDeferred += h.nExact;
    if (deferFrom > 0 && rounds >= deferFrom && h.nPairs > h.nDecided && h.nPairs - h.nDecided <= deferMax) nUndecDeferredUpper += (i64)(h.nPairs - h.nDecided);
    if (account("round")) return -1;
    nU = h.nU;
    int* t = Ucur; Ucur = Unext; Unext = t;
  }
  hipLaunchKernelGGL(k_keep, dim3(sd::div_up(N, 256)), dim3(256), 0, s, state, d_keep, N);
  SD_LAUNCH_CHECK();
  SD_CHECK(hipStreamSynchronize(s));
  if (stats) { stats[0] = totalPairs; stats[1] = totalExact; stats[2] = rounds; stats[3] = totalNbr;
               stats[4] = (int64_t)ns_pairs; stats[5] = n_pair_launches; stats[6] = (int64_t)ns_full; stats[7] = (int64_t)ns_pre;
               stats[8] = totalSpill; stats[9] = totalDecided; stats[10] = totalUndecDeferred; }
  if (verbose) {
    printf("NMS: %lld pair intersections (%lld on the exact-join path), %d greedy rounds, %lld neighbour entries\n",
           (long long)totalPairs, (long long)totalExact, rounds, (long long)totalNbr);
    fflush(stdout);
  }
  return 0;
}

namespace {
__global__ void __launch_bounds__(256) k_old_build(const int* __restrict__ polys, int N, int R, int* __restrict__ vx, int* __restrict__ vy,
                                                   int4* __restrict__ bbox, float* __restrict__ area, int* __restrict__ gmax) {
  const int i = blockIdx.x * blockDim.x + threadIdx.x;
  if (i >= N) return;
  const int* py = polys + (size_t)i * 2 * R;
  const int* px = py + R;
  int x1 = 0, x2 = 0, y1 = 0, y2 = 0;
  float a = 0.f;
  for (int k = 0; k < R; ++k) {
    const int y = py[k], x = px[k];
    if (k == 0) { x1 = x2 = x; y1 = y2 = y; }
    else { x1 = x < x1 ? x : x1; x2 = x > x2 ? x : x2; y1 = y < y1 ? y : y1; y2 = y > y2 ? y : y2; }
    vx[(size_t)i * R + k] = x; vy[(size_t)i * R + k] = y;
    const int kn = (k + 1 == R) ? 0 : k + 1;
    a += (float)((i64)x * py[kn] - (i64)y * px[kn]);
  }
  area[i] = (float)(0.5 * (double)fabsf(a));
  bbox[i] = make_int4(x1, x2, y1, y2);
  atomicMax(&gmax[0], x2 - x1); atomicMax(&gmax[1], y2 - y1);
}
struct OldSearch { int max_bbox_search, grid_y, grid_x, height, width; };
template <int MODE>
__global__ void __launch_bounds__(256) k_old_pairs(int N, OldSearch o, const int* __restrict__ mapping, const int4* __restrict__ bbox,
                                                   const int* __restrict__ gmax, int* __restrict__ cnt, const i64* __restrict__ start,
                                                   int2* __restrict__ pairs) {
  const int lane = threadIdx.x & 63;
  const int i = blockIdx.x * (blockDim.x >> 6) + (threadIdx.x >> 6);
  if (i >= N) return;
  const int4 bi = bbox[i];
  const i64 base = MODE ? start[i] : 0;
  int n = 0;
  auto visit = [&](bool in, int j) {
    const bool hit = in && j > i && j < N && bbox_intersect(bi, bbox[j]);
    const unsigned long long m = __ballot(hit);
    if (MODE && hit) pairs[base + n + __popcll(m & ((1ull << lane) - 1))] = make_int2(i, j);
    n += __popcll(m);
  };
  if (o.max_bbox_search) {
    const int mx = gmax[0], my = gmax[1];
    const int xs = max((bi.x - mx) / o.grid_x, 0), xe = min((bi.y + mx) / o.grid_x, o.width);
    const int ys = max((bi.z - my) / o.grid_y, 0), ye = min((bi.w + my) / o.grid_y, o.height);
    const int w = xe - xs, h = ye - ys;
    if (w > 0 && h > 0) {
      const i64 tot = (i64)w * h;
      for (i64 t = 0; t < tot; t += 64) {
        const i64 q = t + lane;
        const bool in = q < tot;
        int j = -1;
        if (in) { const int jj = ys + (int)(q / w), ii = xs + (int)(q % w); j = mapping[(size_t)jj * o.width + ii]; }
        visit(in, j);
      }
    }
  } else {
    for (int t = i + 1; t < N; t += 64) visit(t + lane < N, t + lane);
  }
  if (!MODE && lane == 0) cnt[i] = n;
}
__global__ void __launch_bounds__(1024) k_old_replay(int N, const i64* __restrict__ start, const int2* __restrict__ pairs,
                                                     const unsigned char* __restrict__ supp, volatile unsigned char* state) {
  for (int i = 0; i < N; ++i) {
    const i64 beg = start[i], end = start[i + 1];
    if (beg == end) continue;
    if (state[i] != ST_SUPPRESSED)
      for (i64 t = beg + threadIdx.x; t < end; t += blockDim.x) if (supp[t]) state[pairs[t].y] = ST_SUPPRESSED;
    __threadfence_block();
    __syncthreads();
  }
}
}

extern "C" int sd_nms2d_old_device(const int32_t* d_polys, int n_polys, int n_rays, const int32_t* d_mapping, int height, int width,
                                   float threshold, int max_bbox_search, int grid_y, int grid_x, int verbose, uint8_t* d_keep,
                                   void* stream_) {
  hipStream_t s = (hipStream_t)stream_;
  const int N = n_polys, R = n_rays;
  if (N <= 0) return 0;
  if (R < 1 || R > 256) { sd::set_error("sd_nms2d_old: n_rays=%d unsupported (1..256)", R); return -1; }
  if (max_bbox_search && (!d_mapping || height <= 0 || width <= 0 || grid_y <= 0 || grid_x <= 0)) {
    sd::set_error("sd_nms2d_old: max_bbox_search needs a (height, width) mapping and positive grid steps"); return -1;
  }
  if (verbose) {
    printf("Non Maximum Suppression (2D) ++++ \n");
    printf("NMS: n_polys  = %d \nNMS: n_rays   = %d  \nNMS: thresh   = %.3f \nNMS: max_bbox_search = %d \n", N, R, threshold, max_bbox_search);
    printf("NMS: using HIP (gfx950), every candidate pair by the scan-beam pair kernel, greedy order replayed on the device\n");
  }
  sd::Arena& A = sd::arena();
  if (A.begin(s)) return -1;
  int* vx = A.take_n<int>((size_t)N * R);
  int* vy = A.take_n<int>((size_t)N * R);
  int4* bbox = A.take_n<int4>(N);
  float* area = A.take_n<float>(N);
  int* gmax = A.take_n<int>(2);
  unsigned char* state = A.take_n<unsigned char>(N);
  int* cnt = A.take_n<int>(N + 1);
  i64* start = A.take_n<i64>(N + 1);
  Counters* d_cnt = (Counters*)A.take(sizeof(Counters));
  if (!vx || !vy || !bbox || !area || !gmax || !state || !cnt || !start || !d_cnt) return -1;
  SD_CHECK(hipMemsetAsync(gmax, 0, 2 * sizeof(int), s));
  SD_CHECK(hipMemsetAsync(state, 0, N, s));
  SD_CHECK(hipMemsetAsync(cnt, 0, (N + 1) * sizeof(int), s));
  SD_CHECK(hipMemsetAsync(d_cnt, 0, sizeof(Counters), s));
  hipLaunchKernelGGL(k_old_build, dim3(sd::div_up(N, 256)), dim3(256), 0, s, d_polys, N, R, vx, vy, bbox, area, gmax);
  SD_LAUNCH_CHECK();
  const OldSearch o{max_bbox_search, grid_y, grid_x, height, width};
  hipLaunchKernelGGL((k_old_pairs<0>), dim3(sd::div_up(N, 4)), dim3(256), 0, s, N, o, d_mapping, bbox, gmax, cnt, (const i64*)nullptr, (int2*)nullptr);
  SD_LAUNCH_CHECK();
  size_t tmpBytes = 0;
  (void)hipcub::DeviceScan::ExclusiveSum(nullptr, tmpBytes, cnt, start, N + 1, s);
  void* scanTmp = A.take(tmpBytes + 256);
  if (!scanTmp) return -1;
  SD_CHECK(hipcub::DeviceScan::ExclusiveSum(scanTmp, tmpBytes, cnt, start, N + 1, s));
  i64 total = 0;
  SD_CHECK(hipMemcpyAsync(&total, start + N, sizeof(i64), hipMemcpyDeviceToHost, s));
  SD_CHECK(hipStreamSynchronize(s));
  if (total < 0 || total >= (i64)(1ll << 30)) {
    sd::set_error("sd_nms2d_old: %lld candidate pairs exceed the capacity of one call (2^30)", (long long)total); return -1;
  }
  if (total > 0) {
    const unsigned int qCap = (unsigned int)total + 64u;
    int2* pairs = A.take_n<int2>((size_t)total + 64);
    unsigned char* supp = A.take_n<unsigned char>((size_t)total + 64);
    unsigned int* spillPairs = A.take_n<unsigned int>(qCap);
    unsigned int* exactPairs = A.take_n<unsigned int>(qCap);
    size_t prepStride;
    if (R <= 32) prepStride = sizeof(sdclip::PolyPrep<32>); else if (R <= 64) prepStride = sizeof(sdclip::PolyPrep<64>);
    else if (R <= 128) prepStride = sizeof(sdclip::PolyPrep<128>); else prepStride = sizeof(sdclip::PolyPrep<256>);
    void* prep = A.take((size_t)N * prepStride);
    if (!pairs || !supp || !spillPairs || !exactPairs || !prep) return -1;
    SD_CHECK(hipMemsetAsync(supp, 0, (size_t)total + 64, s));
    hipLaunchKernelGGL((k_old_pairs<1>), dim3(sd::div_up(N, 4)), dim3(256), 0, s, N, o, d_mapping, bbox, gmax, cnt, (const i64*)start, pairs);
    SD_LAUNCH_CHECK();
    const unsigned long long nP = (unsigned long long)total;
    SD_CHECK(hipMemcpyAsync(&d_cnt->nPairs, &nP, sizeof(nP), hipMemcpyHostToDevice, s));
    PairQueues q1{spillPairs, &d_cnt->nSpill, exactPairs, &d_cnt->nExact, qCap};
    PairQueues q2{exactPairs, &d_cnt->nExact, exactPairs, &d_cnt->nExact, qCap};
    int rc;
    const unsigned int* none = nullptr;
    if (R <= 32) {
      rc = BeamPath<32, 64>::prepare(vx, vy, N, R, prep, s);
      if (!rc) rc = BeamPath<32, 64>::tier1(pairs, none, &d_cnt->nPairs, none, prep, area, threshold, state, supp, q1, s);
      if (!rc) rc = BeamPath<32, 64>::tier2(pairs, spillPairs, &d_cnt->nSpill, none, prep, area, threshold, state, supp, q2, s);
    } else if (R <= 64) {
      rc = BeamPath<64, 64>::prepare(vx, vy, N, R, prep, s);
      if (!rc) rc = BeamPath<64, 64>::tier2(pairs, none, &d_cnt->nPairs, none, prep, area, threshold, state, supp, q2, s);
    } else if (R <= 128) {
      rc = BeamPath<128, 32>::prepare(vx, vy, N, R, prep, s);
      if (!rc) rc = BeamPath<128, 32>::tier2(pairs, none, &d_cnt->nPairs, none, prep, area, threshold, state, supp, q2, s);
    } else {
      rc = BeamPath<256, 16>::prepare(vx, vy, N, R, prep, s);
      if (!rc) rc = BeamPath<256, 16>::tier2(pairs, none, &d_cnt->nPairs, none, prep, area, threshold, state, supp, q2, s);
    }
    if (rc) return -1;
    if (sd::clip_full_pairs(pairs, exactPairs, &d_cnt->nExact, qCap, R, vx, vy, area, threshold, state, supp, &d_cnt->nErr, s)) return -1;
    hipLaunchKernelGGL(k_old_replay, dim3(1), dim3(1024), 0, s, N, (const i64*)start, (const int2*)pairs, (const unsigned char*)supp, state);
    SD_LAUNCH_CHECK();
    Counters h;
    SD_CHECK(hipMemcpyAsync(&h, d_cnt, sizeof(Counters), hipMemcpyDeviceToHost, s));
    SD_CHECK(hipStreamSynchronize(s));
    if (h.nSpill > qCap || h.nExact > qCap) { sd::set_error("sd_nms2d_old: pair queue overflow (internal error)"); return -1; }
    if (h.nErr) { sd::set_error("sd_nms2d_old: %u pairs exceeded the general path's fixed capacities", h.nErr); return -1; }
  }
  hipLaunchKernelGGL(k_keep, dim3(sd::div_up(N, 256)), dim3(256), 0, s, state, d_keep, N);
  SD_LAUNCH_CHECK();
  SD_CHECK(hipStreamSynchronize(s));
  if (verbose) { printf("NMS: %lld candidate pairs evaluated\n", (long long)total); fflush(stdout); }
  return 0;
}

extern "C" int sd_nms2d_old_host(const int32_t* polys, int n_polys, int n_rays, const int32_t* mapping, int height, int width,
                                 float threshold, int max_bbox_search, int grid_y, int grid_x, int verbose, uint8_t* keep) {
  if (n_polys <= 0) return 0;
  int32_t *d_polys = nullptr, *d_map = nullptr;
  uint8_t* d_keep = nullptr;
  const size_t pb = (size_t)n_polys * 2 * n_rays * sizeof(int32_t), mb = max_bbox_search ? (size_t)height * width * sizeof(int32_t) : 0;
  SD_CHECK(hipMalloc(&d_polys, pb));
  if (mb) SD_CHECK(hipMalloc(&d_map, mb));
  SD_CHECK(hipMalloc(&d_keep, n_polys));
  int rc = -1;
  do {
    if (hipMemcpy(d_polys, polys, pb, hipMemcpyHostToDevice) != hipSuccess) { sd::set_error("H2D failed"); break; }
    if (mb && hipMemcpy(d_map, mapping, mb, hipMemcpyHostToDevice) != hipSuccess) { sd::set_error("H2D failed"); break; }
    if (sd_nms2d_old_device(d_polys, n_polys, n_rays, d_map, height, width, threshold, max_bbox_search, grid_y, grid_x, verbose, d_keep, nullptr)) break;
    if (hipMemcpy(keep, d_keep, n_polys, hipMemcpyDeviceToHost) != hipSuccess) { sd::set_error("D2H failed"); break; }
    rc = 0;
  } while (0);
  (void)hipFree(d_polys); if (d_map) (void)hipFree(d_map); (void)hipFree(d_keep);
  return rc;
}

extern "C" int sd_nms2d_host(const float* dist, const float* points, int n_polys, int n_rays, int use_kdtree, int use_bbox,
                             int verbose, float threshold, uint8_t* keep, int64_t* stats) {
  if (n_polys <= 0) return 0;
  float *d_dist = nullptr, *d_pts = nullptr;
  uint8_t* d_keep = nullptr;
  SD_CHECK(hipMalloc(&d_dist, (size_t)n_polys * n_rays * sizeof(float)));
  SD_CHECK(hipMalloc(&d_pts, (size_t)n_polys * 2 * sizeof(float)));
  SD_CHECK(hipMalloc(&d_keep, n_polys));
  int rc = -1;
  do {
    if (hipMemcpy(d_dist, dist, (size_t)n_polys * n_rays * sizeof(float), hipMemcpyHostToDevice) != hipSuccess) { sd::set_error("H2D failed"); break; }
    if (hipMemcpy(d_pts, points, (size_t)n_polys * 2 * sizeof(float), hipMemcpyHostToDevice) != hipSuccess) { sd::set_error("H2D failed"); break; }
    if (sd_nms2d_device(d_dist, d_pts, n_polys, n_rays, use_kdtree, use_bbox, verbose, threshold, d_keep, stats, nullptr)) break;
    if (hipMemcpy(keep, d_keep, n_polys, hipMemcpyDeviceToHost) != hipSuccess) { sd::set_error("D2H failed"); break; }
    rc = 0;
  } while (0);
  (void)hipFree(d_dist); (void)hipFree(d_pts); (void)hipFree(d_keep);
  return rc;
}
```

### stardist_amd/csrc/nms_rounds.h

```cpp
#pragma once
#include "common.h"
#include <hipcub/hipcub.hpp>

namespace {

enum { ST_UNDECIDED = 0, ST_KEPT = 1, ST_SUPPRESSED = 2 };

#define WAIT_NONE (-2)
#define WAIT_SCAN (-1)

struct NmsFlags { int use_kdtree, use_bbox, thr_nonneg; float thr, max_dist; };

__global__ void k_iota(int* a, int n) { int i = blockIdx.x * blockDim.x + threadIdx.x; if (i < n) a[i] = i; }
__global__ void k_keep(const unsigned char* __restrict__ state, unsigned char* __restrict__ keep, int n) {
  int i = blockIdx.x * blockDim.x + threadIdx.x;
  if (i < n) keep[i] = (state[i] != ST_SUPPRESSED);
}

__global__ void __launch_bounds__(256) k_sum_halves(const int* __restrict__ nLow, const int* __restrict__ nHigh, int N, unsigned long long* total) {
  __shared__ unsigned long long ws[4];
  unsigned long long v = 0;
  for (int i = blockIdx.x * 256 + threadIdx.x; i < N; i += gridDim.x * 256) v += (unsigned long long)(nLow[i] + nHigh[i]);
  for (int o = 32; o; o >>= 1) v += __shfl_xor(v, o);
  if ((threadIdx.x & 63) == 0) ws[threadIdx.x >> 6] = v;
  __syncthreads();
  if (threadIdx.x == 0) atomicAdd(total, ws[0] + ws[1] + ws[2] + ws[3]);
}

__global__ void __launch_bounds__(1024) k_round_triage(const int* __restrict__ U, int nU, const unsigned char* __restrict__ state,
                                                       const int* __restrict__ waitOn, int* __restrict__ Unext, int* __restrict__ K,
                                                       int* __restrict__ S, int* counters ,
                                                       const unsigned char* __restrict__ pend) {
  const int t = blockIdx.x * blockDim.x + threadIdx.x;
  const int lane = threadIdx.x & 63, wave = threadIdx.x >> 6, nw = blockDim.x >> 6;
  int kind = 0, i = -1;
  if (t < nU) {
    i = U[t];
    if (state[i] != ST_SUPPRESSED) {
      const int wo = waitOn[i];
      if (pend && pend[i]) kind = 1;
      else if (wo == WAIT_NONE) kind = 2;
      else if (wo >= 0 && state[wo] == ST_UNDECIDED) kind = 1;
      else kind = 3;
    }
  }
  __shared__ int wcnt[3][16];
  __shared__ int bbase[3];
#pragma unroll
  for (int q = 1; q <= 3; ++q) {
    const unsigned long long m = __ballot(kind == q);
    if (lane == 0) wcnt[q - 1][wave] = __popcll(m);
  }
  __syncthreads();
  if (threadIdx.x < 3) {
    int sum = 0;
    for (int w = 0; w < nw; ++w) { const int c = wcnt[threadIdx.x][w]; wcnt[threadIdx.x][w] = sum; sum += c; }
    bbase[threadIdx.x] = sum ? atomicAdd(&counters[threadIdx.x], sum) : 0;
  }
  __syncthreads();
#pragma unroll
  for (int q = 1; q <= 3; ++q) {
    const unsigned long long m = __ballot(kind == q);
    if (kind == q) (q == 1 ? Unext : (q == 2 ? K : S))[bbase[q - 1] + wcnt[q - 1][wave] + __popcll(m & ((1ull << lane) - 1))] = i;
  }
}

__global__ void __launch_bounds__(256) k_round_scan(const int* __restrict__ S, const unsigned char* __restrict__ state,
                                                    const long long* __restrict__ nbrStart, const int* __restrict__ nbrLow, const int* __restrict__ nbr,
                                                    int* __restrict__ waitOn, int* __restrict__ Unext, int* __restrict__ K,
                                                    int* counters , const unsigned char* __restrict__ pend) {
  const int lane = threadIdx.x & 63;
  const int nS = counters[2];
  const int nWaves = gridDim.x * (blockDim.x >> 6);
  int myI = -1, myKind = 0, nbuf = 0;
  auto flush = [&]() {
#pragma unroll
    for (int q = 1; q <= 2; ++q) {
      const unsigned long long m = __ballot(lane < nbuf && myKind == q);
      if (!m) continue;
      int base = 0;
      if (lane == 0) base = atomicAdd(&counters[q - 1], __popcll(m));
      base = __shfl(base, 0);
      if (lane < nbuf && myKind == q) (q == 1 ? Unext : K)[base + __popcll(m & ((1ull << lane) - 1))] = myI;
    }
    nbuf = 0;
  };
  const int sub = lane >> 4, sl = lane & 15;
  for (int w0 = (blockIdx.x * (blockDim.x >> 6) + (threadIdx.x >> 6)) * 4; w0 < nS; w0 += nWaves * 4) {
    const int w = w0 + sub;
    const bool valid = w < nS;
    const int i = valid ? S[w] : -1;
    long long t = 0, end = 0;
    if (valid) { t = nbrStart[i]; end = t + nbrLow[i]; }
    int found = -1;
    while (__any(found < 0 && t < end)) {
      const long long idx = t + sl;
      int j = -1;
      if (found < 0 && idx < end) { j = nbr[idx]; if (!(j < i && state[j] == ST_UNDECIDED)) j = -1; }
      const unsigned long long m = __ballot(j >= 0);
      const unsigned int m16 = (unsigned int)(m >> (sub << 4)) & 0xffffu;
      const int src = (sub << 4) + (m16 ? __ffs((int)m16) - 1 : 0);
      const int jf = __shfl(j, src);
      if (found < 0 && m16) found = jf;
      t += 16;
    }
    if (valid && sl == 0) waitOn[i] = found >= 0 ? found : WAIT_NONE;
    const int kind = (found >= 0 || (valid && pend && pend[i])) ? 1 : 2;
#pragma unroll
    for (int q = 0; q < 4; ++q) {
      const int vi = __shfl(i, q << 4), vk = __shfl(kind, q << 4);
      if (vi >= 0) { if (lane == nbuf) { myI = vi; myKind = vk; } ++nbuf; }
    }
    if (nbuf > 60) flush();
  }
  flush();
}

struct NbrLists {
  int* count; int* low; long long* start;
  int* nbr; int* waitOn;
  long long total, slotTotal;
  bool slots;
};

template <class LaunchNeighbours, class BeforeLists>
int build_neighbour_lists(sd::Arena& A, hipStream_t s, int N, bool singlePass, void* scanTmp, size_t scanBytes,
                          LaunchNeighbours launch, BeforeLists beforeLists, NbrLists& L) {
  L.nbr = nullptr; L.waitOn = nullptr; L.total = 0; L.slotTotal = 0; L.slots = false;
  if (singlePass) {
    SD_CHECK(hipcub::DeviceScan::ExclusiveSum(scanTmp, scanBytes, L.count, L.start, N + 1, s));
    SD_CHECK(hipMemcpyAsync(&L.slotTotal, L.start + N, sizeof(long long), hipMemcpyDeviceToHost, s));
    SD_CHECK(hipStreamSynchronize(s));
    L.slots = L.slotTotal >= 0 && L.slotTotal < 0x7fffffffll;
  }
  if (L.slots) {
    L.nbr = A.take_n<int>((size_t)L.slotTotal);
    if (!L.nbr) L.slots = false;
  }
  if (L.slots && beforeLists()) return -1;
  if (!L.slots) {
    SD_CHECK(hipMemsetAsync(L.count, 0, (N + 1) * sizeof(int), s));
    launch(0, L);
    SD_LAUNCH_CHECK();
    SD_CHECK(hipcub::DeviceScan::ExclusiveSum(scanTmp, scanBytes, L.count, L.start, N + 1, s));
    SD_CHECK(hipMemcpyAsync(&L.total, L.start + N, sizeof(long long), hipMemcpyDeviceToHost, s));
    SD_CHECK(hipStreamSynchronize(s));
    if (beforeLists()) return -1;
  }
  if (L.total < 0 || L.total >= 0x7fffffffll) return 1;
  if (!L.slots) L.nbr = A.take_n<int>((size_t)L.total);
  L.waitOn = A.take_n<int>(N);
  if (!L.nbr || !L.waitOn) return -1;
  if (L.slots) {
    unsigned long long* d_total = A.take_n<unsigned long long>(1);
    if (!d_total) return -1;
    SD_CHECK(hipMemsetAsync(d_total, 0, sizeof(unsigned long long), s));
    launch(2, L);
    hipLaunchKernelGGL(k_sum_halves, dim3(sd::div_up(N, 256) < 1024 ? sd::div_up(N, 256) : 1024), dim3(256), 0, s, L.low, L.count, N, d_total);
    SD_LAUNCH_CHECK();
    unsigned long long tot = 0;
    SD_CHECK(hipMemcpyAsync(&tot, d_total, sizeof(tot), hipMemcpyDeviceToHost, s));
    SD_CHECK(hipStreamSynchronize(s));
    L.total = (long long)tot;
  } else {
    launch(1, L);
    SD_LAUNCH_CHECK();
  }
  return 0;
}

}
```

### stardist_amd/lib/_native.py

```python
import ctypes
import os

import numpy as np

_HERE = os.path.dirname(os.path.abspath(__file__))
LIB_PATH = os.path.join(_HERE, "..", "csrc", "libstardist_hip.so")

_lib = None
last_stats = {}

_c_f32p = ctypes.POINTER(ctypes.c_float)
_c_i32p = ctypes.POINTER(ctypes.c_int32)
_c_i64p = ctypes.POINTER(ctypes.c_int64)
_c_u8p = ctypes.POINTER(ctypes.c_uint8)
_c_u16p = ctypes.POINTER(ctypes.c_uint16)
_vp = ctypes.c_void_p
_i = ctypes.c_int
_f = ctypes.c_float

SIGNATURES = {
    "sd_last_error": (ctypes.c_char_p, []),
    "sd_version": (_i, []),
    "sd_device_count": (_i, []),
    "sd_release_workspace": (_i, []),
    "sd_set_option": (_i, [ctypes.c_char_p, _i]),
    "sd_get_option": (_i, [ctypes.c_char_p]),
    "sd_nms2d_host": (_i, [_vp, _vp, _i, _i, _i, _i, _i, _f, _vp, _vp]),
    "sd_nms2d_device": (_i, [_vp, _vp, _i, _i, _i, _i, _i, _f, _vp, _vp, _vp]),
    "sd_nms2d_old_host": (_i, [_vp, _i, _i, _vp, _i, _i, _f, _i, _i, _i, _i, _vp]),
    "sd_nms2d_old_device": (_i, [_vp, _i, _i, _vp, _i, _i, _f, _i, _i, _i, _i, _vp, _vp]),
    "sd_clip_pairs_device": (_i, [_vp, _vp, _vp, _vp, _i, _i, _vp, _vp, _vp]),
    "sd_area_bounds_pairs_device": (_i, [_vp, _vp, _vp, _vp, _i, _i, _vp, _vp, _vp, _vp]),
    "sd_prepare_polys_device": (_i, [_vp, _vp, _i, _i, _vp, ctypes.c_int64, _vp]),
    "sd_poly_pass_device": (_i, [_vp, _vp, _i, _i, _vp, _vp, _vp]),
    "sd_star_dist2d_host": (_i, [_vp, _i, _i, _i, _i, _i, _vp]),
    "sd_star_dist2d_device": (_i, [_vp, _i, _i, _i, _i, _i, _vp, _vp]),
    "sd_star_dist3d_host": (_i, [_vp, _i, _i, _i, _vp, _vp, _vp, _i, _i, _i, _i, _vp]),
    "sd_star_dist3d_device": (_i, [_vp, _i, _i, _i, _vp, _vp, _vp, _i, _i, _i, _i, _vp, _vp]),
    "sd_edt_prob_device": (_i, [_vp, _i, _i, _i, ctypes.c_double, ctypes.c_double, ctypes.c_double, _i, _vp, _vp]),
    "sd_dist_to_coord_device": (_i, [_vp, _vp, _vp, ctypes.c_longlong, _i, ctypes.c_double, ctypes.c_double, _vp, _vp]),
    "sd_polygons_to_label_host": (_i, [_vp, _vp, _i, _i, _i, _i, _vp]),
    "sd_polygons_to_label_device": (_i, [_vp, _vp, _i, _i, _i, _i, _vp, _vp]),
    "sd_polygons_to_label_window_device": (_i, [_vp, _vp, _i, _i, _i, _i, _i, _i, _i, _i, _vp, _vp]),
    "sd_polyhedron_to_label_window_device": (_i, [_vp, _vp, _vp, _vp, _i, _i, _i, _vp] + [_i] * 13 + [_vp, _vp]),
    "_LIB_non_maximum_suppression_sparse": (None, [_vp, _vp, _vp, _i, _i, _i, _vp, _vp, _f, _i, _i, _i, _vp]),
    "sd_nms3d_device": (_i, [_vp, _vp, _vp, _i, _i, _i, _vp, _vp, _f, _i, _i, _i, _vp, _vp, _vp]),
    "sd_hiv_pairs_device": (_i, [_vp, _vp, _i, _i, _i, _vp, _vp, _vp, _i, _vp, _vp, _vp]),
    "_LIB_polyhedron_to_label": (None, [_vp, _vp, _vp, _vp, _i, _i, _i, _vp, _i, _i, _i, _i, _i, _i, _i, _vp]),
    "sd_polyhedron_to_label_device": (_i, [_vp, _vp, _vp, _vp, _i, _i, _i, _vp, _i, _i, _i, _i, _i, _i, _i, _vp, _vp]),
    "sd_select_candidates_device": (_i, [_vp, _vp, _i, _vp, _vp, _i, _f, _i, _vp, _vp, _vp, _vp, _vp]),
    "sd_survivor_positions_device": (_i, [_vp, ctypes.c_longlong, _vp, _vp, _vp]),
    "sd_survivors2d_device": (_i, [_vp, _i, _vp, _vp, _vp, _i, _vp, _vp, _vp, _vp, _vp, _vp, _vp]),
    "sd_sorted_rows_device": (_i, [_vp, _vp, _i, _i, _vp, _vp, _vp, _vp, _vp, _vp, _vp]),
    "sd_sort_scores_desc_device": (_i, [_vp, _i, _vp, _vp, _vp]),
    "sd_bias_act_device": (_i, [_vp, _vp, ctypes.c_longlong, _i, ctypes.c_longlong, _i, _vp]),
    "sd_add_bias_act_device": (_i, [_vp, _vp, _vp, ctypes.c_longlong, _i, ctypes.c_longlong, _i, _vp]),
    "sd_maxpool_ndhwc_device": (_i, [_vp, _i, _i, _i, _i, _i, _i, _i, _vp, _vp]),
    "sd_upcat_ndhwc_device": (_i, [_vp, _i, _i, _vp, _i, _i, _i, _i, _vp, _vp]),
    "sd_inside_polyhedron_device": (_i, [_vp, _vp, _i, _i, _vp, _vp, _vp, ctypes.c_longlong, _i, _vp, _vp]),
    "sd_bias_act_dot_device": (_i, [_vp, _vp, _vp, ctypes.c_longlong, _i, _i, _vp, _vp, _i, _vp, _vp]),
    "sd_head_rows_device": (_i, [_vp, _i, _vp, ctypes.c_longlong, _vp, _vp, _i, ctypes.c_float, _vp, _vp]),
    "sd_conv3_packed_floats": (ctypes.c_longlong, [_i, _i, _i]),
    "sd_conv3_pack_weights_host": (_i, [_vp, _i, _i, _i, _vp]),
    "sd_conv3_ndhwc_device": (_i, [_vp, _i, _i, _i, _vp, _i, _i, _i, _i, _i, _i, _i, _vp, _vp, _i, _i, _vp, _vp]),
    "sd_conv3_res_ndhwc_device": (_i, [_vp, _i, _i, _i, _vp, _i, _i, _i, _i, _i, _i, _i, _vp, _vp, _vp, _i, _i, _i, _vp, _vp]),
    "sd_conv3_bf16x6_res_ndhwc_device": (_i, [_vp, _i, _i, _i, _vp, _i, _i, _i, _i, _i, _i, _i, _vp, _vp, _vp, _i, _i, _i, _vp, _vp]),
    "sd_convg_packed_floats": (ctypes.c_longlong, [_i, _i, _i, _i, _i]),
    "sd_convg_pack_weights_host": (_i, [_vp, _i, _i, _i, _i, _i, _vp]),
    "sd_convg_ndhwc_device": (_i, [_vp] + [_i] * 17 + [_vp, _vp, _vp, _i, _i, _i, _vp, _i, _vp]),
    "sd_conv3_bf16x6_packed_floats": (ctypes.c_longlong, [_i, _i, _i]),
    "sd_conv3_bf16x6_pack_weights_host": (_i, [_vp, _i, _i, _i, _vp]),
    "sd_conv3_bf16x6_ndhwc_device": (_i, [_vp, _i, _i, _i, _vp, _i, _i, _i, _i, _i, _i, _i, _vp, _vp, _i, _i, _vp, _vp]),
    "sd_conv3_f16x3_packed_floats": (ctypes.c_longlong, [_i, _i, _i]),
    "sd_conv3_f16x3_pack_weights_host": (_i, [_vp, _i, _i, _i, _vp]),
    "sd_conv3_f16x3_ndhwc_device": (_i, [_vp, _i, _i, _i, _vp, _i, _i, _i, _i, _i, _i, _i, _vp, _vp, _i, _i, _vp, _vp, _vp]),
    "sd_conv3_f16x3_res_ndhwc_device": (_i, [_vp, _i, _i, _i, _vp, _i, _i, _i, _i, _i, _i, _i, _vp, _vp, _vp, _i, _i, _i, _vp, _vp, _vp]),
    "sd_conv3_f16x3_dot_ndhwc_device": (_i, [_vp, _i, _i, _i, _vp, _i, _i, _i, _i, _i, _i, _i, _vp, _vp, _i, _i, _vp, _vp, _vp, _vp, _vp]),
    "sd_dot_combine_device": (_i, [_vp, _i, ctypes.c_longlong, _vp, _i, _vp, _vp]),
    "sd_conv3_f16x3_fmt_ndhwc_device": (_i, [_vp, _i, _i, _vp, _i, _i, _i, _i, _i, _i, _vp, _vp, _i, _i, _vp, _i, _i, _vp, _vp, _vp, _vp]),
    "sd_conv3_f16x3_rows_device": (_i, [_vp, _i, _i, _i, _i, _i, _i, _vp, _vp, _i, _i, _vp, ctypes.c_longlong, _vp, _vp]),
    "sd_conv3_c1x32_split16_device": (_i, [_vp, _i, _i, _i, _i, _vp, _vp, _i, _vp, _vp, _vp]),
    "sd_maxpool_split16_ndhwc_device": (_i, [_vp, _i, _i, _i, _i, _i, _i, _i, _vp, _vp]),
    "sd_split16_pack_device": (_i, [_vp, ctypes.c_longlong, _i, _vp, _vp, _vp]),
    "sd_split16_unpack_device": (_i, [_vp, ctypes.c_longlong, _i, _vp, _vp]),
    "sd_label_overlap_device": (_i, [_vp, _vp, ctypes.c_longlong, ctypes.c_longlong, _vp, _vp, _vp, _vp, _vp]),
    "sd_label_overlap_stack_device": (_i, [_vp, _i, ctypes.c_longlong, ctypes.c_longlong, _vp, _vp, _vp, _vp, _vp, _vp]),
    "sd_relabel_stack_device": (_i, [_vp, _i, ctypes.c_longlong, _vp, _vp, _vp, _vp, _vp, _vp]),
    "sd_conv_wgrad_ndhwc_device": (_i, [_vp, _i, _vp, _i, _i, _vp, _i, _i, _i, _i, _i, _i, _vp, _vp, _vp]),
    "sd_relu_mask_device": (_i, [_vp, _vp, ctypes.c_longlong, _vp, _vp]),
    "sd_maxpool_adjoint_ndhwc_device": (_i, [_vp, _vp, _i, _i, _i, _i, _i, _i, _vp, _vp]),
    "sd_upcat_adjoint_ndhwc_device": (_i, [_vp, _i, _i, _i, _i, _i, _i, _vp, _vp, _vp]),
    "sd_stardist_loss2d_device": (_i, [_vp, _vp, _vp, _vp, ctypes.c_longlong, _i, _i, ctypes.c_double, ctypes.c_double, ctypes.c_double,
                                       _vp, _vp, _vp, _vp]),
    "sd_stardist_loss2d_metrics_device": (_i, [_vp, _vp, _vp, _vp, ctypes.c_longlong, _i, _i, ctypes.c_double, ctypes.c_double,
                                               ctypes.c_double, _vp, _vp, _vp, _vp, _vp]),
    "sd_conv3_wgrad_ndhwc_device": (_i, [_vp, _i, _vp, _i, _i, _vp, _i, _i, _i, _i, _i, _i, _vp, _vp, _vp]),
    "sd_convg_wgrad_ndhwc_device": (_i, [_vp, _i, _vp, _i] + [_i] * 16 + [_vp, _vp, _vp]),
    "sd_convg_dgrad_ndhwc_device": (_i, [_vp, _i, _vp, _i] + [_i] * 16 + [_vp, _vp]),
    "sd_maxpool3d_adjoint_ndhwc_device": (_i, [_vp, _vp, _i, _i, _i, _i, _i, _i, _i, _i, _vp, _vp]),
    "sd_upcat3d_adjoint_ndhwc_device": (_i, [_vp, _i, _i, _i, _i, _i, _i, _i, _vp, _vp, _vp]),
    "sd_class_targets_device": (_i, [_vp, _i, _i, _i, _i, _vp, _vp, _vp, _vp, _vp, _vp, _i, _i, _i, _vp, _i, _vp, _vp, _vp]),
    "sd_class_loss_device": (_i, [_vp, _vp, _vp, ctypes.c_longlong, _i, ctypes.c_double, _vp, _vp, _vp]),
    "sd_percentiles_device": (_i, [_vp, _i, ctypes.c_longlong, _i, _vp, _i, _i, _vp, _vp]),
    "sd_normalize_mi_ma_device": (_i, [_vp, _i, ctypes.c_longlong, _i, _vp, _vp, _f, _i, _vp, _vp]),
    "_LIB_non_maximum_suppression_2d": (None, [_vp, _vp, _i, _i, _f, _i, _i, _i, _vp]),
    "_LIB_polygon_to_label": (None, [_vp, _vp, _i, _i, _i, _i, _vp]),
    "_LIB_star_dist": (None, [_vp, _i, _i, _i, _i, _i, _vp]),
    "_LIB_star_dist3d": (None, [_vp, _i, _i, _i, _vp, _vp, _vp, _i, _i, _i, _i, _vp]),
}


class NativeError(RuntimeError):
    pass


def lib():
    global _lib
    if _lib is None:
        path = os.path.abspath(LIB_PATH)
        if not os.path.exists(path):
            raise NativeError("libstardist_hip.so not built (%s): run `python -m stardist_amd.build` "
                              "or __graft_entry__.build(); there is no CPU fallback" % path)
        try:
            import torch
        except Exception:
            pass
        l = ctypes.CDLL(path)
        for name, (res, args) in SIGNATURES.items():
            fn = getattr(l, name)
            fn.restype = res
            fn.argtypes = args
        _lib = l
    return _lib


class option(object):

    def __init__(self, name, value):
        self.name, self.value = name.encode(), int(value)

    def __enter__(self):
        self.old = lib().sd_get_option(self.name)
        check(lib().sd_set_option(self.name, self.value))
        return self

    def __exit__(self, *exc):
        lib().sd_set_option(self.name, self.old)
        return False


def require_device():
    if lib().sd_device_count() < 1:
        raise NativeError("no HIP device visible: the stardist_amd natives only run on a GPU "
                          "(there is no CPU fallback)")


def check(rc):
    if rc != 0:
        raise NativeError(lib().sd_last_error().decode(errors="replace"))


def ptr(a):
    if a is None:
        return None
    assert a.flags["C_CONTIGUOUS"]
    return a.ctypes.data_as(ctypes.c_void_p)


def is_torch(x):
    return type(x).__module__.startswith("torch")


def tptr(t):
    assert t.is_cuda and t.is_contiguous()
    return ctypes.c_void_p(t.data_ptr())


def current_stream(device=None):
    import torch
    return ctypes.c_void_p(torch.cuda.current_stream(device).cuda_stream)


def dcall(t, name, *args):
    import torch
    with torch.cuda.device(t.device):
        check(getattr(lib(), name)(*args, current_stream(t.device)))


def on_device_of(t):
    import torch
    return torch.cuda.device(t.device)
```

### stardist_amd/lib/stardist2d.py

```python
import numpy as np

from . import _native as N


def c_non_max_suppression_inds(dist, points, use_kdtree, use_bbox, verbose, threshold, return_stats=False, _as_uint8=False):
    N.require_device()
    stats = np.zeros(16, np.int64)
    if N.is_torch(dist):
        import torch
        assert dist.dtype == torch.float32 and points.dtype == torch.float32
        dist = dist.contiguous(); points = points.contiguous()
        n, R = dist.shape
        keep = torch.empty(n, dtype=torch.uint8, device=dist.device)
        N.dcall(dist, "sd_nms2d_device", N.tptr(dist), N.tptr(points), n, R, int(use_kdtree), int(use_bbox),
                                        int(verbose), float(threshold), N.tptr(keep), N.ptr(stats))
        if not _as_uint8:
            keep = keep.bool()
    else:
        dist = np.ascontiguousarray(dist, np.float32)
        points = np.ascontiguousarray(points, np.float32)
        if dist.ndim != 2 or points.ndim != 2 or points.shape[1] != 2 or len(points) != len(dist):
            raise ValueError("dist must be (n,n_rays) and points (n,2)")
        n, R = dist.shape
        keep = np.zeros(n, np.uint8)
        N.check(N.lib().sd_nms2d_host(N.ptr(dist), N.ptr(points), n, R, int(use_kdtree), int(use_bbox),
                                      int(verbose), float(threshold), N.ptr(keep), N.ptr(stats)))
        keep = keep.astype(bool)
    N.last_stats["nms2d"] = stats
    return (keep, stats) if return_stats else keep


def c_non_max_suppression_inds_old(polys, mapping, threshold, max_bbox_search, grid_y, grid_x, verbose):
    N.require_device()
    if N.is_torch(polys):
        import torch
        assert polys.dtype == torch.int32 and polys.dim() == 3 and polys.shape[1] == 2
        polys = polys.contiguous()
        mapping = mapping.to(torch.int32).contiguous()
        n, _, R = polys.shape
        H, W = (int(mapping.shape[0]), int(mapping.shape[1])) if mapping.dim() == 2 else (0, 0)
        keep = torch.empty(n, dtype=torch.uint8, device=polys.device)
        if n:
            N.dcall(polys, "sd_nms2d_old_device", N.tptr(polys), n, R, N.tptr(mapping) if mapping.numel() else None, H, W, float(threshold),
                    int(max_bbox_search), int(grid_y), int(grid_x), int(verbose), N.tptr(keep))
        return keep.bool()
    polys = np.ascontiguousarray(polys)
    mapping = np.ascontiguousarray(mapping)
    if polys.dtype != np.int32 or mapping.dtype != np.int32:
        raise TypeError("polys and mapping must be int32")
    if polys.ndim != 3 or polys.shape[1] != 2:
        raise ValueError("polys must be (n, 2, n_rays)")
    n, _, R = polys.shape
    H, W = (mapping.shape[0], mapping.shape[1]) if mapping.ndim == 2 else (0, 0)
    keep = np.zeros(n, np.uint8)
    if n:
        N.check(N.lib().sd_nms2d_old_host(N.ptr(polys), n, R, N.ptr(mapping) if mapping.size else None, int(H), int(W), float(threshold),
                                          int(max_bbox_search), int(grid_y), int(grid_x), int(verbose), N.ptr(keep)))
    return keep.astype(bool)


def c_star_dist(src, n_rays, grid_y, grid_x):
    N.require_device()
    n_rays, grid_y, grid_x = int(n_rays), int(grid_y), int(grid_x)
    if N.is_torch(src):
        import torch
        assert src.dtype in (torch.uint16, torch.int16) and src.dim() == 2
        src = src.contiguous()
        H, W = src.shape
        dst = torch.empty(((H - 1) // grid_y + 1, (W - 1) // grid_x + 1, n_rays), dtype=torch.float32, device=src.device)
        N.dcall(src, "sd_star_dist2d_device", N.tptr(src), H, W, n_rays, grid_y, grid_x, N.tptr(dst))
        return dst
    src = np.ascontiguousarray(src)
    if src.dtype != np.uint16:
        src = src.astype(np.uint16)
    H, W = src.shape
    dst = np.empty(((H - 1) // grid_y + 1, (W - 1) // grid_x + 1, n_rays), np.float32)
    N.check(N.lib().sd_star_dist2d_host(N.ptr(src), H, W, n_rays, grid_y, grid_x, N.ptr(dst)))
    return dst


def c_polygons_to_label(coord, labels, shape, window=None):
    N.require_device()
    H, W = int(shape[0]), int(shape[1])
    if N.is_torch(coord):
        import torch
        coord = coord.contiguous().float()
        labels = labels.contiguous().to(torch.int32)
        n, _, R = coord.shape
        (y0, x0), (h, w) = ((0, 0), (H, W)) if window is None else window
        out = torch.empty((int(h), int(w)), dtype=torch.int32, device=coord.device)
        N.dcall(coord, "sd_polygons_to_label_window_device", N.tptr(coord), N.tptr(labels), n, R, H, W, int(y0), int(x0), int(h), int(w), N.tptr(out))
        return out
    if window is not None:
        raise ValueError("window rendering takes device tensors")
    coord = np.ascontiguousarray(coord, np.float32)
    labels = np.ascontiguousarray(labels, np.int32)
    n = coord.shape[0]
    R = coord.shape[2] if coord.ndim == 3 else 0
    out = np.zeros((H, W), np.int32)
    if n:
        N.check(N.lib().sd_polygons_to_label_host(N.ptr(coord), N.ptr(labels), n, R, H, W, N.ptr(out)))
    return out


def survivors_of_sorted(keep, prob, points, dist, want_paint=True):
    import torch
    from ..geometry.geom2d import ray_angles, _SC_CACHE
    N.require_device()
    assert keep.is_cuda and prob.dtype == torch.float32 and dist.dtype == torch.float32 and points.dtype == torch.int64 and points.shape[1] == 2
    n, R = int(dist.shape[0]), int(dist.shape[1])
    assert keep.numel() == n == prob.numel() == points.shape[0]
    dev = keep.device
    keep = keep.contiguous().view(torch.uint8) if keep.dtype == torch.bool else keep.contiguous()
    prob, points, dist = prob.contiguous(), points.contiguous(), dist.contiguous()
    pos = torch.empty(max(n, 1), dtype=torch.int64, device=dev)
    cnt = torch.empty(1, dtype=torch.int32, device=dev)
    N.dcall(keep, "sd_survivor_positions_device", N.tptr(keep), n, N.tptr(pos), N.tptr(cnt))
    m = int(cnt.item())
    key = (R, str(dev))
    sct = _SC_CACHE.get(key)
    if sct is None:
        phis = ray_angles(R)
        sct = _SC_CACHE[key] = torch.as_tensor(np.ascontiguousarray(np.array([np.sin(phis), np.cos(phis)])), device=dev)
    oprob = torch.empty(m, dtype=torch.float32, device=dev)
    opts = torch.empty((m, 2), dtype=torch.int64, device=dev)
    coord = torch.empty((m, 2, R), dtype=torch.float32, device=dev)
    cpaint = torch.empty((m, 2, R), dtype=torch.float32, device=dev) if want_paint else None
    lpaint = torch.empty(m, dtype=torch.int32, device=dev) if want_paint else None
    if m:
        N.dcall(keep, "sd_survivors2d_device", N.tptr(pos), m, N.tptr(prob), N.tptr(points), N.tptr(dist), R, N.tptr(sct), N.tptr(oprob), N.tptr(opts),
                N.tptr(coord), N.tptr(cpaint) if want_paint else None, N.tptr(lpaint) if want_paint else None)
    return oprob, opts, coord, cpaint, lpaint


def clip_pairs(xa, ya, xb, yb):
    import torch
    N.require_device()
    dev = torch.device("cuda")
    t = [torch.from_numpy(np.ascontiguousarray(v, np.int32)).to(dev) for v in (xa, ya, xb, yb)]
    n, R = t[0].shape
    out = torch.zeros(n, dtype=torch.int64, device=dev)
    fl = torch.zeros(n, dtype=torch.int32, device=dev)
    N.dcall(t[0], "sd_clip_pairs_device", N.tptr(t[0]), N.tptr(t[1]), N.tptr(t[2]), N.tptr(t[3]), n, R,
                                         N.tptr(out), N.tptr(fl))
    torch.cuda.synchronize()
    return out.cpu().numpy(), fl.cpu().numpy()


def area_bounds_pairs(xa, ya, xb, yb):
    import torch
    N.require_device()
    dev = torch.device("cuda")
    t = [torch.from_numpy(np.ascontiguousarray(v, np.int32)).to(dev) for v in (xa, ya, xb, yb)]
    n, R = t[0].shape
    area = torch.zeros(n, dtype=torch.float32, device=dev); band = torch.zeros(n, dtype=torch.float32, device=dev)
    info = torch.zeros(n, dtype=torch.int32, device=dev)
    N.dcall(t[0], "sd_area_bounds_pairs_device", N.tptr(t[0]), N.tptr(t[1]), N.tptr(t[2]), N.tptr(t[3]), n, R, N.tptr(area), N.tptr(band), N.tptr(info))
    torch.cuda.synchronize()
    info = info.cpu().numpy()
    return area.cpu().numpy(), band.cpu().numpy(), (info & 1).astype(bool), (info >> 8) & 0x3FF, (info >> 18) & 0x7FF
```

Measured before the change: 305.8.

## Restructure NMS build, store only lower neighbours, skip pairs with suppressed partner

The per-polygon build kernel now puts one thread on each polygon and stages distance rows and vertex outputs through shared memory with vectorised copies. It also reduces the global stats per block before the atomics. The neighbour lists now hold only lower-index neighbours. The emit kernel recomputes higher-index candidates from the cell grid instead of reading stored lists, and pairs whose partner is already suppressed are marked decided and skipped. This cuts neighbour-list memory and traffic and avoids intersection work that is no longer needed, at the cost of repeating the grid window walks every round and more serial work per thread in the build. A new build entry point is exposed for testing.

```diff
diff --git a/include/stardist_hip.h b/include/stardist_hip.h
--- a/include/stardist_hip.h
+++ b/include/stardist_hip.h
@@ -21,6 +21,9 @@
 int sd_nms2d_device(const float* d_dist, const float* d_points, int n_polys, int n_rays,
                     int use_kdtree, int use_bbox, int verbose, float threshold,
                     uint8_t* d_keep, int64_t* stats, void* stream);
+
+int sd_nms2d_build_device(const float* d_dist, const float* d_points, int n_polys, int n_rays, int32_t* d_vx, int32_t* d_vy,
+                          int32_t* d_bbox, float* d_radius, float* d_area, int32_t* d_gstats, void* stream);
 
 int sd_nms2d_old_host(const int32_t* polys, int n_polys, int n_rays, const int32_t* mapping, int height, int width,
                       float threshold, int max_bbox_search, int grid_y, int grid_x, int verbose, uint8_t* keep);
diff --git a/stardist_amd/csrc/nms2d.hip b/stardist_amd/csrc/nms2d.hip
--- a/stardist_amd/csrc/nms2d.hip
+++ b/stardist_amd/csrc/nms2d.hip
@@ -78,64 +78,87 @@
   }
 }
 
-__global__ void __launch_bounds__(256) k_build32(const float* __restrict__ dist, const float* __restrict__ pts,
-                                                 const float2* __restrict__ sincos, int N, int R,
-                                                 int* __restrict__ vx, int* __restrict__ vy, int4* __restrict__ bbox,
-                                                 float* __restrict__ radius, float* __restrict__ area, int* gstats) {
-  __shared__ int sxy[8][2][32];
-  const int l = threadIdx.x & 31, hw = threadIdx.x >> 5;
-  const int i = blockIdx.x * 8 + hw;
-  const bool cv = i < N, lv = cv && l < R;
-  int* sx = sxy[hw][0];
-  int* sy = sxy[hw][1];
-  float py = 0.f, px = 0.f;
-  if (cv) { py = pts[2 * i]; px = pts[2 * i + 1]; }
-  float xmin = INFINITY, xmax = -INFINITY, ymin = INFINITY, ymax = -INFINITY, rmax = 0.f;
-  if (lv) {
-    const float d = dist[(size_t)i * R + l];
-    const float2 sc = sincos[l];
-    const float y = py + d * sc.x;
-    const float x = px + d * sc.y;
-    xmin = xmax = x; ymin = ymax = y;
-    const int X = (int)(long long)x, Y = (int)(long long)y;
-    sx[l] = X; sy[l] = Y;
-    vx[(size_t)i * R + l] = X; vy[(size_t)i * R + l] = Y;
-    rmax = fmaxf(0.f, d);
-  }
-  for (int o = 16; o; o >>= 1) {
-    xmin = fminf(xmin, __shfl_xor(xmin, o)); xmax = fmaxf(xmax, __shfl_xor(xmax, o));
-    ymin = fminf(ymin, __shfl_xor(ymin, o)); ymax = fmaxf(ymax, __shfl_xor(ymax, o));
-    rmax = fmaxf(rmax, __shfl_xor(rmax, o));
-  }
-  __builtin_amdgcn_wave_barrier();
-  i64 s = 0, sa = 0;
-  if (lv) {
-    const int kn = (l + 1 == R) ? 0 : l + 1;
-    const i64 c = (i64)sx[l] * sy[kn] - (i64)sy[l] * sx[kn];
-    s = c; sa = (c < 0 ? -c : c);
-  }
-  for (int o = 16; o; o >>= 1) { s += __shfl_xor(s, o); sa += __shfl_xor(sa, o); }
-  if (cv && l == 0) {
+__global__ void __launch_bounds__(64) k_build32(const float* __restrict__ dist, const float* __restrict__ pts,
+                                                const float2* __restrict__ sincos, int N, int R, int vec4,
+                                                int* __restrict__ vx, int* __restrict__ vy, int4* __restrict__ bbox,
+                                                float* __restrict__ radius, float* __restrict__ area, int* gstats) {
+  extern __shared__ __attribute__((aligned(16))) int rows[];
+  __shared__ float2 ssc[32];
+  const int c = threadIdx.x;
+  const int base = blockIdx.x * 64;
+  const int cnt = min(64, N - base);
+  const int nel = cnt * R;
+  int* sx = rows;
+  int* sy = rows + 64 * R;
+  if (c < R) ssc[c] = sincos[c];
+  {
+    const int* g = (const int*)dist + (size_t)base * R;
+    const int nv = vec4 ? nel >> 2 : 0;
+    for (int e = c; e < nv; e += 64) ((int4*)rows)[e] = ((const int4*)g)[e];
+    for (int e = 4 * nv + c; e < nel; e += 64) rows[e] = g[e];
+  }
+  __syncthreads();
+  const bool cv = c < cnt;
+  float rmax = 0.f;
+  int iy = INT32_MAX, ix = INT32_MAX, iyh = INT32_MIN, ixh = INT32_MIN;
+  if (cv) {
+    const int i = base + c;
+    const float py = pts[2 * i], px = pts[2 * i + 1];
+    float xmin = INFINITY, xmax = -INFINITY, ymin = INFINITY, ymax = -INFINITY;
+    i64 s = 0, sa = 0;
+    int X0 = 0, Y0 = 0, Xp = 0, Yp = 0;
+    int k = c % R;
+    for (int t = 0; t < R; ++t) {
+      const float d = __int_as_float(rows[c * R + k]);
+      const float2 sc = ssc[k];
+      const float y = py + d * sc.x;
+      const float x = px + d * sc.y;
+      xmin = fminf(xmin, x); xmax = fmaxf(xmax, x);
+      ymin = fminf(ymin, y); ymax = fmaxf(ymax, y);
+      rmax = fmaxf(rmax, d);
+      const int X = (int)(long long)x, Y = (int)(long long)y;
+      sx[c * R + k] = X; sy[c * R + k] = Y;
+      if (t) { const i64 cr = (i64)Xp * Y - (i64)Yp * X; s += cr; sa += (cr < 0 ? -cr : cr); }
+      else { X0 = X; Y0 = Y; }
+      Xp = X; Yp = Y;
+      k = (k + 1 == R) ? 0 : k + 1;
+    }
+    { const i64 cr = (i64)Xp * Y0 - (i64)Yp * X0; s += cr; sa += (cr < 0 ? -cr : cr); }
     float a;
     if (sa < (1ll << 24)) a = (float)s;
     else {
       a = 0.f;
-      for (int k = 0; k < R; ++k) {
-        const int kn = (k + 1 == R) ? 0 : k + 1;
-        a += (float)((i64)sx[k] * sy[kn] - (i64)sy[k] * sx[kn]);
+      for (int q = 0; q < R; ++q) {
+        const int qn = (q + 1 == R) ? 0 : q + 1;
+        a += (float)((i64)sx[c * R + q] * sy[c * R + qn] - (i64)sy[c * R + q] * sx[c * R + qn]);
       }
     }
     area[i] = (float)(0.5 * (double)fabsf(a));
     radius[i] = rmax;
     bbox[i] = make_int4((int)xmin, (int)xmax, (int)ymin, (int)ymax);
+    iy = iyh = (int)floorf(py); ix = ixh = (int)floorf(px);
+  }
+  for (int o = 32; o; o >>= 1) {
+    rmax = fmaxf(rmax, __shfl_xor(rmax, o));
+    iy = min(iy, __shfl_xor(iy, o)); iyh = max(iyh, __shfl_xor(iyh, o));
+    ix = min(ix, __shfl_xor(ix, o)); ixh = max(ixh, __shfl_xor(ixh, o));
+  }
+  if (c == 0) {
     const int rb = __float_as_int(rmax);
-    const int iy = (int)floorf(py), ix = (int)floorf(px);
     volatile int* gs = gstats;
     if (rb > gs[0]) atomicMax(&gstats[0], rb);
     if (iy < gs[1]) atomicMin(&gstats[1], iy);
-    if (iy > gs[2]) atomicMax(&gstats[2], iy);
+    if (iyh > gs[2]) atomicMax(&gstats[2], iyh);
     if (ix < gs[3]) atomicMin(&gstats[3], ix);
-    if (ix > gs[4]) atomicMax(&gstats[4], ix);
+    if (ixh > gs[4]) atomicMax(&gstats[4], ixh);
+  }
+  __syncthreads();
+  {
+    int* gx = vx + (size_t)base * R;
+    int* gy = vy + (size_t)base * R;
+    const int nv = vec4 ? nel >> 2 : 0;
+    for (int e = c; e < nv; e += 64) { ((int4*)gx)[e] = ((const int4*)sx)[e]; ((int4*)gy)[e] = ((const int4*)sy)[e]; }
+    for (int e = 4 * nv + c; e < nel; e += 64) { gx[e] = sx[e]; gy[e] = sy[e]; }
   }
 }
 
@@ -183,6 +206,7 @@
     int u = -1;
     for (int yy = w.ylo; yy <= w.yhi; ++yy) u += cellStart[yy * g.nx + w.xhi + 1] - cellStart[yy * g.nx + w.xlo];
     slotCap[i] = u;
+    if (i == 0) slotCap[N] = 0;
   }
 }
 
@@ -207,10 +231,39 @@
   return ok;
 }
 
+struct WindowRuns { int rbeg, excl, nrows, total; };
+__device__ __forceinline__ WindowRuns window_runs(const GridP g, const Window win, const int* __restrict__ cellStart, int lane) {
+  WindowRuns w;
+  w.nrows = __builtin_amdgcn_readfirstlane(win.yhi - win.ylo + 1);
+  int rbeg = 0, rlen = 0;
+  if (lane < w.nrows) { rbeg = cellStart[(win.ylo + lane) * g.nx + win.xlo]; rlen = cellStart[(win.ylo + lane) * g.nx + win.xhi + 1] - rbeg; }
+  int incl = rlen;
+  for (int o = 1; o < MAX_WIN_ROWS; o <<= 1) { const int t = __shfl_up(incl, o); if (lane >= o) incl += t; }
+  w.total = __builtin_amdgcn_readlane(incl, w.nrows - 1);
+  w.rbeg = rbeg; w.excl = incl - rlen;
+  return w;
+}
+template <class Body>
+__device__ __forceinline__ void walk_window(const WindowRuns& w, int lane, Body&& body) {
+  int r0 = 0;
+  for (int t = 0; t < w.total; t += 64) {
+    while (r0 + 1 < w.nrows && __builtin_amdgcn_readlane(w.excl, r0 + 1) <= t) ++r0;
+    int rb = __builtin_amdgcn_readlane(w.rbeg, r0), re = __builtin_amdgcn_readlane(w.excl, r0);
+    const int v = t + lane;
+    for (int r = r0 + 1; r < w.nrows; ++r) {
+      const int e_r = __builtin_amdgcn_readlane(w.excl, r);
+      if (e_r > t + 63) break;
+      const int b_r = __builtin_amdgcn_readlane(w.rbeg, r);
+      if (e_r <= v) { rb = b_r; re = e_r; }
+    }
+    body(v < w.total ? rb + (v - re) : -1);
+  }
+}
+
 template <int MODE>
 __global__ void __launch_bounds__(256) k_neighbours(int N, GridP g, NmsFlags f, const CellRec* __restrict__ rec, const int* __restrict__ cellStart,
                                                     int* __restrict__ nbrCount, int* __restrict__ nbrLow, const i64* __restrict__ nbrStart,
-                                                    int* __restrict__ nbr, int* __restrict__ waitOn, int by_bbox, float reach, unsigned long long* __restrict__ total) {
+                                                    int* __restrict__ nbr, int* __restrict__ waitOn, int by_bbox, float reach) {
   const int wave = threadIdx.x >> 6, lane = threadIdx.x & 63;
   const int per = gridDim.x >> 3;
   const int blk = (blockIdx.x & 7) * per + (blockIdx.x >> 3);
@@ -218,50 +271,26 @@
   if (w >= N) return;
   const CellRec me = rec[w];
   const int i = me.j;
-  int cy, cx;
-  cell_of(g, me.py, me.px, cy, cx);
   const int4 bi = me.bb;
   const float pyi = me.py, pxi = me.px, ai = me.area;
-  int nLo = 0, nHi = 0;
+  int nLo = 0;
   int minj = INT32_MAX;
-  const i64 baseLo = MODE ? nbrStart[i] : 0;
-  const i64 baseHi = MODE == 1 ? baseLo + nbrLow[i] : (MODE == 2 ? nbrStart[i + 1] - 1 : 0);
-  const Window win = cell_window(g, by_bbox != 0, reach, bi, pyi, pxi);
-  const int nrows = win.yhi - win.ylo + 1;
-  int rbeg = 0, rlen = 0;
-  if (lane < nrows) { rbeg = cellStart[(win.ylo + lane) * g.nx + win.xlo]; rlen = cellStart[(win.ylo + lane) * g.nx + win.xhi + 1] - rbeg; }
-  int incl = rlen;
-  for (int o = 1; o < MAX_WIN_ROWS; o <<= 1) { const int t = __shfl_up(incl, o); if (lane >= o) incl += t; }
-  const int total_recs = __shfl(incl, nrows - 1);
-  const int excl = incl - rlen;
-  for (int t = 0; t < total_recs; t += 64) {
-    const int v = t + lane;
+  const i64 base = MODE ? nbrStart[i] : 0;
+  const WindowRuns runs = window_runs(g, cell_window(g, by_bbox != 0, reach, bi, pyi, pxi), cellStart, lane);
+  walk_window(runs, lane, [&](int ri) {
     bool hit = false;
     int j = -1;
-    {
-      int rb = 0, re = 0;
-      for (int r = 0; r < nrows; ++r) {
-        const int e_r = __shfl(excl, r), b_r = __shfl(rbeg, r);
-        if (e_r <= v) { rb = b_r; re = e_r; }
-      }
-      if (v < total_recs) {
-        const CellRec r = rec[rb + (v - re)];
-        j = r.j;
-        if (j != i) hit = may_interact(f, bi, r.bb, pyi, pxi, r.py, r.px, ai, r.area);
-      }
-    }
-    const unsigned long long mLo = __ballot(hit && j < i), mHi = __ballot(hit && j > i);
-    if (MODE && hit) {
-      const unsigned long long below = (1ull << lane) - 1;
-      if (j < i) { nbr[baseLo + nLo + __popcll(mLo & below)] = j; if (j < minj) minj = j; }
-      else if (MODE == 1) nbr[baseHi + nHi + __popcll(mHi & below)] = j;
-      else nbr[baseHi - (nHi + __popcll(mHi & below))] = j;
-    }
-    nLo += __popcll(mLo); nHi += __popcll(mHi);
-  }
-  if (!MODE && lane == 0) { nbrCount[i] = nLo + nHi; nbrLow[i] = nLo; }
-  if (MODE == 2 && lane == 0) nbrLow[i] = nLo;
-  if (MODE && lane == 0) nbrCount[i] = nHi;
+    if (ri >= 0) {
+      const CellRec r = rec[ri];
+      j = r.j;
+      if (j < i) hit = may_interact(f, bi, r.bb, pyi, pxi, r.py, r.px, ai, r.area);
+    }
+    const unsigned long long m = __ballot(hit);
+    if (MODE && hit) { nbr[base + nLo + __popcll(m & ((1ull << lane) - 1))] = j; if (j < minj) minj = j; }
+    nLo += __popcll(m);
+  });
+  if (!MODE && lane == 0) nbrCount[i] = nLo;
+  if (MODE != 1 && lane == 0) nbrLow[i] = nLo;
   if (MODE) {
     for (int o = 32; o; o >>= 1) minj = min(minj, __shfl_xor(minj, o));
     if (lane == 0) waitOn[i] = (minj < i) ? minj : WAIT_NONE;
@@ -270,8 +299,8 @@
 
 constexpr int EMIT_STAGE = 512;
 __global__ void __launch_bounds__(256) k_round_emit(const int* __restrict__ K, const int* __restrict__ nKPtr, unsigned char* __restrict__ state,
-                                                    const i64* __restrict__ nbrStart, const int* __restrict__ nbrHigh, const int* __restrict__ nbr, NmsFlags f,
-                                                    const float* __restrict__ pts, const int4* __restrict__ bbox,
+                                                    GridP g, const CellRec* __restrict__ rec, const int* __restrict__ cellStart, int by_bbox, float reach,
+                                                    NmsFlags f, const float* __restrict__ pts, const int4* __restrict__ bbox,
                                                     const float* __restrict__ radius, const float* __restrict__ area,
                                                     int2* __restrict__ pairs, unsigned long long* pairCount,
                                                     unsigned long long pairCap) {
@@ -290,46 +319,45 @@
     nst = 0;
   };
   for (int w = blockIdx.x * (blockDim.x >> 6) + wave; w < nK; w += gridDim.x * (blockDim.x >> 6)) {
-  const int i = K[w];
-  if (lane == 0) state[i] = ST_KEPT;
-  const i64 end = nbrStart[i + 1], beg = end - nbrHigh[i];
-  const int4 bi = bbox[i];
-  const float pyi = pts[2 * i], pxi = pts[2 * i + 1];
-  const float rad = f.max_dist + radius[i];
-  const float rad2 = rad * rad;
-  for (i64 t = beg; t < end; t += 64) {
-    const i64 idx = t + lane;
-    bool emit = false;
-    int j = -1;
-    if (idx < end) {
-      j = nbr[idx];
-      if (j > i && state[j] == ST_UNDECIDED) {
-        bool ok = true;
-        if (f.use_kdtree) {
-          const float d0 = pyi - pts[2 * j], d1 = pxi - pts[2 * j + 1];
+    const int i = K[w];
+    if (lane == 0) state[i] = ST_KEPT;
+    const int4 bi = bbox[i];
+    const float pyi = pts[2 * i], pxi = pts[2 * i + 1];
+    const double ai = (double)area[i] + 1.e-10;
+    const float rad = f.max_dist + radius[i];
+    const float rad2 = rad * rad;
+    const WindowRuns runs = window_runs(g, cell_window(g, by_bbox != 0, reach, bi, pyi, pxi), cellStart, lane);
+    walk_window(runs, lane, [&](int ri) {
+      bool emit = false;
+      int j = -1;
+      if (ri >= 0) {
+        const CellRec r = rec[ri];
+        j = r.j;
+        bool ok = j > i;
+        if (ok && f.use_kdtree) {
+          const float d0 = pyi - r.py, d1 = pxi - r.px;
           float d2 = d0 * d0; d2 += d1 * d1;
           ok = d2 < rad2;
         }
         if (ok && (f.use_bbox || f.thr_nonneg)) {
-          const int4 bj = bbox[j];
+          const int4 bj = r.bb;
           ok = bbox_intersect(bi, bj);
           if (ok && f.thr_nonneg) {
             const double w = (double)(min(bi.y, bj.y) - max(bi.x, bj.x)), hgt = (double)(min(bi.w, bj.w) - max(bi.z, bj.z));
-            const float ub = (float)((w * hgt) / fmin((double)area[i] + 1.e-10, (double)area[j] + 1.e-10));
+            const float ub = (float)((w * hgt) / fmin(ai, (double)r.area + 1.e-10));
             if (!(ub > f.thr)) ok = false;
           }
         }
-        emit = ok;
+        emit = ok && state[j] == ST_UNDECIDED;
       }
-    }
-    const unsigned long long m = __ballot(emit);
-    if (m) {
-      const int c = __popcll(m);
-      if (nst + c > EMIT_STAGE) flush();
-      if (emit) stage[wave][nst + __popcll(m & ((1ull << lane) - 1))] = make_int2(i, j);
-      nst += c;
-    }
-  }
+      const unsigned long long m = __ballot(emit);
+      if (m) {
+        const int c = __popcll(m);
+        if (nst + c > EMIT_STAGE) flush();
+        if (emit) stage[wave][nst + __popcll(m & ((1ull << lane) - 1))] = make_int2(i, j);
+        nst += c;
+      }
+    });
   }
   flush();
 }
@@ -512,13 +540,24 @@
   }
 }
 __global__ void k_tail_init2(Deferred d, const unsigned char* __restrict__ kind, int2* __restrict__ pairs, unsigned int* __restrict__ exact,
-                             unsigned long long* nPairs, unsigned int* nExact, unsigned int* firstNew, unsigned char* __restrict__ decided) {
+                             unsigned long long* nPairs, unsigned int* nExact, unsigned int* firstNew, unsigned char* __restrict__ decided,
+                             const unsigned char* __restrict__ state, unsigned int* __restrict__ nSkipped) {
   unsigned int n = *d.count; if (n > d.cap) n = d.cap;
   for (unsigned int t = blockIdx.x * blockDim.x + threadIdx.x; t < n; t += gridDim.x * blockDim.x) {
-    pairs[t] = d.pairs[t];
-    if (kind[t] == 0) { exact[atomicAdd(nExact, 1u)] = t; decided[t] = 3; } else decided[t] = 0;
+    const int2 ij = d.pairs[t];
+    pairs[t] = ij;
+    if (kind[t] == 0) { exact[atomicAdd(nExact, 1u)] = t; decided[t] = 3; }
+    else if (state[ij.y] == ST_SUPPRESSED) { decided[t] = 4; atomicAdd(nSkipped, 1u); }
+    else decided[t] = 0;
   }
   if (blockIdx.x == 0 && threadIdx.x == 0) { *nPairs = n; *firstNew = n; }
+}
+__global__ void k_round_lists_init(int N, int* __restrict__ U, unsigned char* __restrict__ state, unsigned char* __restrict__ pend,
+                                   int* __restrict__ head, unsigned int* __restrict__ dcount) {
+  const int i = blockIdx.x * blockDim.x + threadIdx.x;
+  if (i == 0) *dcount = 0;
+  if (i >= N) return;
+  U[i] = i; state[i] = ST_UNDECIDED; pend[i] = 0; head[i] = -1;
 }
 __global__ void k_copy_u32(unsigned int* dst, const unsigned int* src) { *dst = *src; }
 __device__ __forceinline__ bool deferred_suppresses(int j, const int* __restrict__ defHead, const int* __restrict__ defNext,
@@ -580,6 +619,7 @@
   }
 }
 
+__device__ __forceinline__ bool pair_j_suppressed(const unsigned char* __restrict__ state, int2 ij) { return state && state[ij.y] == ST_SUPPRESSED; }
 constexpr int PAIR_BUCKETS = 4096;
 struct PairKey { const char* prep; size_t prepStride; float inv; int nl, ny, nx; };
 __device__ __forceinline__ int pair_bucket(const float* __restrict__ pts, int2 ij, const PairKey& k) {
@@ -596,15 +636,23 @@
 }
 __global__ void __launch_bounds__(256) k_pair_bucket_count(const int2* __restrict__ pairs, const unsigned long long* __restrict__ nPtr,
                                                            const unsigned int* __restrict__ firstPtr, const float* __restrict__ pts, PairKey key,
-                                                           unsigned int* __restrict__ hist, const unsigned char* __restrict__ decided) {
+                                                           unsigned int* __restrict__ hist, const unsigned char* __restrict__ decided,
+                                                           const unsigned char* __restrict__ state, unsigned int* __restrict__ nSkipped) {
   __shared__ unsigned int h[PAIR_BUCKETS];
+  __shared__ unsigned int skipped;
   for (int b = threadIdx.x; b < PAIR_BUCKETS; b += 256) h[b] = 0;
+  if (threadIdx.x == 0) skipped = 0;
   __syncthreads();
   const unsigned long long n = *nPtr, first = firstPtr ? *firstPtr : 0u;
-  for (unsigned long long t = first + (unsigned long long)blockIdx.x * 256 + threadIdx.x; t < n; t += (unsigned long long)gridDim.x * 256)
-    if (!decided || !decided[t]) atomicAdd(&h[pair_bucket(pts, pairs[t], key)], 1u);
+  for (unsigned long long t = first + (unsigned long long)blockIdx.x * 256 + threadIdx.x; t < n; t += (unsigned long long)gridDim.x * 256) {
+    if (decided && decided[t]) continue;
+    const int2 ij = pairs[t];
+    if (pair_j_suppressed(state, ij)) { atomicAdd(&skipped, 1u); continue; }
+    atomicAdd(&h[pair_bucket(pts, ij, key)], 1u);
+  }
   __syncthreads();
   for (int b = threadIdx.x; b < PAIR_BUCKETS; b += 256) if (h[b]) atomicAdd(&hist[b], h[b]);
+  if (threadIdx.x == 0 && skipped) atomicAdd(nSkipped, skipped);
 }
 __global__ void __launch_bounds__(1024) k_pair_bucket_scan(const unsigned int* __restrict__ hist, unsigned int* __restrict__ cursor,
                                                            unsigned long long* __restrict__ nOrdered) {
@@ -629,11 +677,13 @@
 __global__ void __launch_bounds__(256) k_pair_bucket_scatter(const int2* __restrict__ pairs, const unsigned long long* __restrict__ nPtr,
                                                              const unsigned int* __restrict__ firstPtr, const float* __restrict__ pts, PairKey key,
                                                              unsigned int* __restrict__ cursor, unsigned int* __restrict__ order, unsigned int cap,
-                                                             const unsigned char* __restrict__ decided) {
+                                                             const unsigned char* __restrict__ decided, const unsigned char* __restrict__ state) {
   const unsigned long long n = *nPtr, first = firstPtr ? *firstPtr : 0u;
   for (unsigned long long t = first + (unsigned long long)blockIdx.x * 256 + threadIdx.x; t < n; t += (unsigned long long)gridDim.x * 256) {
     if (decided && decided[t]) continue;
-    const unsigned int k = atomicAdd(&cursor[pair_bucket(pts, pairs[t], key)], 1u);
+    const int2 ij = pairs[t];
+    if (pair_j_suppressed(state, ij)) continue;
+    const unsigned int k = atomicAdd(&cursor[pair_bucket(pts, ij, key)], 1u);
     if (k < cap) order[k] = (unsigned int)t;
   }
 }
@@ -648,7 +698,7 @@
 }
 
 namespace {
-struct Counters { int nU, nK, nS, left; unsigned long long nPairs; unsigned int nSpill, nExact, nErr, nDecided; };
+struct Counters { int nU, nK, nS, left; unsigned long long nPairs; unsigned int nSpill, nExact, nErr, nDecided, nSkipped; };
 
 template <int MAXV, int SPREP>
 struct BeamPath {
@@ -692,6 +742,46 @@
 };
 }
 
+namespace {
+int launch_build(sd::Arena& A, hipStream_t s, const float* d_dist, const float* d_points, int N, int R, int* vx, int* vy, int4* bbox,
+                 float* radius, float* area, int** gstatsOut, hipEvent_t evStart) {
+  const int gs_init[8] = {0, INT32_MAX, INT32_MIN, INT32_MAX, INT32_MIN, 0, 0, 0};
+  std::vector<float> hdr(8 + 2 * (size_t)R);
+  memcpy(hdr.data(), gs_init, sizeof(gs_init));
+  const float ANGLE_PI = 2 * M_PI / R;
+  for (int k = 0; k < R; ++k) { hdr[8 + 2 * k] = sinf(ANGLE_PI * k); hdr[8 + 2 * k + 1] = cosf(ANGLE_PI * k); }
+  int* gstats = A.take_n<int>(8 + 2 * (size_t)R);
+  if (!gstats) return -1;
+  const float2* d_sc = (const float2*)(gstats + 8);
+  SD_CHECK(hipMemcpyAsync(gstats, hdr.data(), hdr.size() * sizeof(float), hipMemcpyHostToDevice, s));
+  if (evStart) SD_CHECK(hipEventRecord(evStart, s));
+  if (R <= 32) {
+    const int vec4 = ((((uintptr_t)d_dist | (uintptr_t)vx | (uintptr_t)vy) & 15) == 0) ? 1 : 0;
+    hipLaunchKernelGGL(k_build32, dim3(sd::div_up(N, 64)), dim3(64), 2 * 64 * (size_t)R * sizeof(int), s, d_dist, d_points, d_sc, N, R, vec4,
+                       vx, vy, bbox, radius, area, gstats);
+  } else
+    hipLaunchKernelGGL(k_build, dim3(sd::div_up(N, 4)), dim3(256), 4 * 2 * R * sizeof(int), s, d_dist, d_points, d_sc, N, R,
+                       vx, vy, bbox, radius, area, gstats);
+  SD_LAUNCH_CHECK();
+  *gstatsOut = gstats;
+  return 0;
+}
+}
+
+extern "C" int sd_nms2d_build_device(const float* d_dist, const float* d_points, int n_polys, int n_rays, int32_t* d_vx, int32_t* d_vy,
+                                     int32_t* d_bbox, float* d_radius, float* d_area, int32_t* d_gstats, void* stream_) {
+  hipStream_t s = (hipStream_t)stream_;
+  if (n_polys <= 0) return 0;
+  if (n_rays < 1 || n_rays > 256) { sd::set_error("sd_nms2d_build: n_rays=%d unsupported (1..256)", n_rays); return -1; }
+  sd::Arena& A = sd::arena();
+  if (A.begin(s)) return -1;
+  int* gstats = nullptr;
+  if (launch_build(A, s, d_dist, d_points, n_polys, n_rays, d_vx, d_vy, (int4*)d_bbox, d_radius, d_area, &gstats, nullptr)) return -1;
+  SD_CHECK(hipMemcpyAsync(d_gstats, gstats, 5 * sizeof(int), hipMemcpyDeviceToDevice, s));
+  SD_CHECK(hipStreamSynchronize(s));
+  return 0;
+}
+
 extern "C" int sd_nms2d_device(const float* d_dist, const float* d_points, int n_polys, int n_rays, int use_kdtree,
                                int use_bbox, int verbose, float threshold, uint8_t* d_keep, int64_t* stats,
                                void* stream_) {
@@ -721,30 +811,16 @@
     return 0;
   }
 
-  std::vector<float2> sc(R);
-  const float ANGLE_PI = 2 * M_PI / R;
-  for (int k = 0; k < R; ++k) { sc[k].x = sinf(ANGLE_PI * k); sc[k].y = cosf(ANGLE_PI * k); }
-  float2* d_sc = A.take_n<float2>(R);
   int* vx = A.take_n<int>((size_t)N * R);
   int* vy = A.take_n<int>((size_t)N * R);
   int4* bbox = A.take_n<int4>(N);
   float* radius = A.take_n<float>(N);
   float* area = A.take_n<float>(N);
-  int* gstats = A.take_n<int>(8);
   unsigned char* state = A.take_n<unsigned char>(N);
   int* candCell = A.take_n<int>(N);
-  if (!d_sc || !vx || !vy || !bbox || !radius || !area || !gstats || !state || !candCell) return -1;
-  SD_CHECK(hipMemcpyAsync(d_sc, sc.data(), R * sizeof(float2), hipMemcpyHostToDevice, s));
-  const int gs_init[8] = {0, INT32_MAX, INT32_MIN, INT32_MAX, INT32_MIN, 0, 0, 0};
-  SD_CHECK(hipMemcpyAsync(gstats, gs_init, sizeof(gs_init), hipMemcpyHostToDevice, s));
-  SD_CHECK(hipMemsetAsync(state, 0, N, s));
-  if (stats) SD_CHECK(hipEventRecord(ev0, s));
-  if (R <= 32)
-    hipLaunchKernelGGL(k_build32, dim3(sd::div_up(N, 8)), dim3(256), 0, s, d_dist, d_points, d_sc, N, R, vx, vy, bbox, radius, area, gstats);
-  else
-    hipLaunchKernelGGL(k_build, dim3(sd::div_up(N, 4)), dim3(256), 4 * 2 * R * sizeof(int), s, d_dist, d_points, d_sc, N, R,
-                       vx, vy, bbox, radius, area, gstats);
-  SD_LAUNCH_CHECK();
+  int* gstats = nullptr;
+  if (!vx || !vy || !bbox || !radius || !area || !state || !candCell) return -1;
+  if (launch_build(A, s, d_dist, d_points, N, R, vx, vy, bbox, radius, area, &gstats, stats ? ev0 : nullptr)) return -1;
   size_t prepStride;
   if (R <= 32) prepStride = sizeof(sdclip::PolyPrep<32>); else if (R <= 64) prepStride = sizeof(sdclip::PolyPrep<64>);
   else if (R <= 128) prepStride = sizeof(sdclip::PolyPrep<128>); else prepStride = sizeof(sdclip::PolyPrep<256>);
@@ -799,16 +875,15 @@
   }
   g.y0 = (float)gs[1]; g.x0 = (float)gs[3]; g.inv_cs = 1.f / cs;
   const int nCells = g.ny * g.nx;
-  int* cellCount = A.take_n<int>(nCells + 1);
+  int* cellCount = A.take_n<int>(2 * ((size_t)nCells + 1));
+  int* cellFill = cellCount ? cellCount + nCells + 1 : nullptr;
   int* cellStart = A.take_n<int>(nCells + 1);
-  int* cellFill = A.take_n<int>(nCells + 1);
   CellRec* cellRec = (CellRec*)A.take((size_t)N * sizeof(CellRec));
   int* nbrCount = A.take_n<int>(N + 1);
   i64* nbrStart = A.take_n<i64>(N + 1);
   int* nbrLow = A.take_n<int>(N + 1);
   if (!cellCount || !cellStart || !cellFill || !cellRec || !nbrCount || !nbrStart || !nbrLow) return -1;
-  SD_CHECK(hipMemsetAsync(cellCount, 0, (nCells + 1) * sizeof(int), s));
-  SD_CHECK(hipMemsetAsync(cellFill, 0, (nCells + 1) * sizeof(int), s));
+  SD_CHECK(hipMemsetAsync(cellCount, 0, 2 * ((size_t)nCells + 1) * sizeof(int), s));
   hipLaunchKernelGGL(k_cell_count, dim3(sd::div_up(N, 256)), dim3(256), 0, s, d_points, N, g, cellCount, candCell);
   SD_LAUNCH_CHECK();
   size_t tmpBytes = 0, tmpBytes2 = 0;
@@ -819,7 +894,6 @@
   if (!scanTmp) return -1;
   SD_CHECK(hipcub::DeviceScan::ExclusiveSum(scanTmp, tmpBytes, cellCount, cellStart, nCells + 1, s));
   const bool singlePass = sd::option(sd::OPT_NMS2D_NBR_SINGLE) != 0;
-  SD_CHECK(hipMemsetAsync(nbrCount, 0, (N + 1) * sizeof(int), s));
   hipLaunchKernelGGL(k_cell_fill, dim3(sd::div_up(N, 256)), dim3(256), 0, s, N, candCell, cellStart, cellFill, d_points, bbox, area, cellRec, g, by_bbox, reach,
                      singlePass ? nbrCount : (int*)nullptr);
   SD_LAUNCH_CHECK();
@@ -828,27 +902,22 @@
   int* head0 = A.take_n<int>(N);
   unsigned int* dcount0 = A.take_n<unsigned int>(1);
   if (!U0 || !pend0 || !head0 || !dcount0) return -1;
-  hipLaunchKernelGGL(k_iota, dim3(sd::div_up(N, 256)), dim3(256), 0, s, U0, N);
-  SD_CHECK(hipMemsetAsync(pend0, 0, N, s));
-  SD_CHECK(hipMemsetAsync(head0, 0xFF, (size_t)N * sizeof(int), s));
-  SD_CHECK(hipMemsetAsync(dcount0, 0, sizeof(unsigned int), s));
+  hipLaunchKernelGGL(k_round_lists_init, dim3(sd::div_up(N, 256)), dim3(256), 0, s, N, U0, state, pend0, head0, dcount0);
 
   NmsFlags f;
   f.use_kdtree = use_kdtree; f.use_bbox = use_bbox; f.thr_nonneg = (threshold >= 0.f); f.thr = threshold; f.max_dist = max_dist;
 
   const int nbBlocks = (sd::div_up(N, 4) + 7) & ~7;
   NbrLists L{};
-  L.count = nbrCount; L.low = nbrLow; L.start = nbrStart;
+  L.count = nbrCount; L.low = nbrLow; L.start = nbrStart; L.lowOnly = true;
   auto launch_neighbours = [&](int mode, const NbrLists& l) {
     if (mode == 0)
       hipLaunchKernelGGL((k_neighbours<0>), dim3(nbBlocks), dim3(256), 0, s, N, g, f, cellRec, cellStart, nbrCount, nbrLow, (const i64*)nullptr, (int*)nullptr,
-                         (int*)nullptr, by_bbox, reach, (unsigned long long*)nullptr);
+                         (int*)nullptr, by_bbox, reach);
     else if (mode == 1)
-      hipLaunchKernelGGL((k_neighbours<1>), dim3(nbBlocks), dim3(256), 0, s, N, g, f, cellRec, cellStart, nbrCount, nbrLow, (const i64*)nbrStart, l.nbr, l.waitOn, by_bbox, reach,
-                         (unsigned long long*)nullptr);
+      hipLaunchKernelGGL((k_neighbours<1>), dim3(nbBlocks), dim3(256), 0, s, N, g, f, cellRec, cellStart, nbrCount, nbrLow, (const i64*)nbrStart, l.nbr, l.waitOn, by_bbox, reach);
     else
-      hipLaunchKernelGGL((k_neighbours<2>), dim3(nbBlocks), dim3(256), 0, s, N, g, f, cellRec, cellStart, nbrCount, nbrLow, (const i64*)nbrStart, l.nbr, l.waitOn, by_bbox, reach,
-                         (unsigned long long*)nullptr);
+      hipLaunchKernelGGL((k_neighbours<2>), dim3(nbBlocks), dim3(256), 0, s, N, g, f, cellRec, cellStart, nbrCount, nbrLow, (const i64*)nbrStart, l.nbr, l.waitOn, by_bbox, reach);
   };
   const int rcLists = build_neighbour_lists(A, s, N, singlePass, scanTmp, tmpBytes, launch_neighbours, launch_side, L);
   if (rcLists > 0) {
@@ -859,7 +928,7 @@
   if (rcLists) return -1;
   const int* nbr = L.nbr;
   int* waitOn = L.waitOn;
-  const i64 totalNbr = L.total;
+  const i64 totalNbr = 2 * L.total;
 
   SD_CHECK(hipStreamWaitEvent(s, evProps, 0));
   if (stats) { SD_CHECK(hipEventRecord(ev1, s)); SD_CHECK(hipEventSynchronize(ev1)); float ms = 0; SD_CHECK(hipEventElapsedTime(&ms, ev0, ev1)); ns_pre = ms * 1e6; }
@@ -880,7 +949,7 @@
   if (!U0 || !U1 || !K || !pairs || !spillPairs || !exactPairs || !Sl || !d_cnt || !bucketHist || !nOrdered || (pairSort && R <= 32 && !pairOrder)) return -1;
   unsigned char* decided = (areaBounds && pairOrder) ? A.take_n<unsigned char>(pairCap) : nullptr;
   if (areaBounds && pairOrder && !decided) return -1;
-  i64 totalDecided = 0;
+  i64 totalDecided = 0, totalSkipped = 0;
   int nU = N, rounds = 0;
   i64 totalPairs = 0, totalExact = 0, totalSpill = 0;
   int* Ucur = U0; int* Unext = U1;
@@ -937,10 +1006,12 @@
           hipLaunchKernelGGL(k_defer_undecided, dim3(256), dim3(256), 0, s, pairs, &d_cnt->nPairs, &d_cnt->nDecided, deferMax, decided, state, dfr, defKind, &d_cnt->nErr);
         const unsigned int* bfirst = (suppOut && deferFrom > 0) ? nullptr : first;
         SD_CHECK(hipStreamWaitEvent(s, evPrep, 0));
-        hipLaunchKernelGGL(k_pair_bucket_count, dim3(512), dim3(256), 0, s, pairs, &d_cnt->nPairs, bfirst, d_points, key, bucketHist, decided);
+        const unsigned char* liveState = suppOut ? nullptr : state;
+        hipLaunchKernelGGL(k_pair_bucket_count, dim3(512), dim3(256), 0, s, pairs, &d_cnt->nPairs, bfirst, d_points, key, bucketHist, decided, liveState,
+                           &d_cnt->nSkipped);
         hipLaunchKernelGGL(k_pair_bucket_scan, dim3(1), dim3(1024), 0, s, bucketHist, bucketHist + PAIR_BUCKETS, nOrdered);
         hipLaunchKernelGGL(k_pair_bucket_scatter, dim3(512), dim3(256), 0, s, pairs, &d_cnt->nPairs, bfirst, d_points, key, bucketHist + PAIR_BUCKETS,
-                           pairOrder, qCap, decided);
+                           pairOrder, qCap, decided, liveState);
         SD_LAUNCH_CHECK();
         rc = BeamPath<32, 64>::tier1(pairs, pairOrder, nOrdered, (const unsigned int*)nullptr, prep, area, threshold, state, suppOut, q1, s);
       } else {
@@ -973,13 +1044,13 @@
   auto account = [&](const char* what) -> int {
     if (h.nPairs > pairCap || h.nSpill > qCap || h.nExact > qCap) { sd::set_error("sd_nms2d: pair queue overflow (internal error)"); return -1; }
     if (h.nErr) { sd::set_error("sd_nms2d: %u pairs exceeded the general path's fixed capacities or the deferred-pair list (with more than 64 rays: at least that many; the launch stops at the first)", h.nErr); return -1; }
-    totalPairs += (i64)h.nPairs; totalExact += h.nExact; totalSpill += h.nSpill; totalDecided += h.nDecided;
+    totalPairs += (i64)h.nPairs; totalExact += h.nExact; totalSpill += h.nSpill; totalDecided += h.nDecided; totalSkipped += h.nSkipped;
     if (stats) {
       float ms = 0, ms2 = 0;
       SD_CHECK(hipEventElapsedTime(&ms, ev0, ev1)); SD_CHECK(hipEventElapsedTime(&ms2, ev2, ev3));
       if (h.nPairs) { ns_pairs += ms * 1e6; ++n_pair_launches; }
       ns_full += ms2 * 1e6;
-      if (sd::option(sd::OPT_TRACE)) printf("%s %d: nU=%d nK=%d pairs=%llu decided by the area enclosure=%u spill=%u exact=%u pair_kernel=%.3f ms general_path=%.3f ms\n", what, rounds, h.nU, h.nK, h.nPairs, h.nDecided, h.nSpill, h.nExact, ms, ms2);
+      if (sd::option(sd::OPT_TRACE)) printf("%s %d: nU=%d nK=%d pairs=%llu decided by the area enclosure=%u j already suppressed=%u spill=%u exact=%u pair_kernel=%.3f ms general_path=%.3f ms\n", what, rounds, h.nU, h.nK, h.nPairs, h.nDecided, h.nSkipped, h.nSpill, h.nExact, ms, ms2);
     }
     return 0;
   };
@@ -993,7 +1064,8 @@
       SD_CHECK(hipMemsetAsync(supp, 0, pairCap, s));
       const int wg = sd::div_up(nU, 4) < 2048 ? sd::div_up(nU, 4) : 2048;
       if (deferFrom > 0) {
-        hipLaunchKernelGGL(k_tail_init2, dim3(64), dim3(256), 0, s, dfr, defKind, pairs, exactPairs, &d_cnt->nPairs, &d_cnt->nExact, firstNew, decided);
+        hipLaunchKernelGGL(k_tail_init2, dim3(64), dim3(256), 0, s, dfr, defKind, pairs, exactPairs, &d_cnt->nPairs, &d_cnt->nExact, firstNew, decided, state,
+                           &d_cnt->nSkipped);
         hipLaunchKernelGGL(k_copy_u32, dim3(1), dim3(1), 0, s, nJoinDef, &d_cnt->nExact);
       } else
         hipLaunchKernelGGL(k_tail_init, dim3(64), dim3(256), 0, s, dfr, pairs, exactPairs, &d_cnt->nPairs, &d_cnt->nExact, firstNew);
@@ -1035,7 +1107,7 @@
     hipLaunchKernelGGL(k_round_triage, dim3(sd::div_up(nU, 1024)), dim3(1024), 0, s, Ucur, nU, state, waitOn, Unext, K, Sl, (int*)d_cnt, dfr.pend);
     const int wgrid = sd::div_up(nU, 4) < 2048 ? sd::div_up(nU, 4) : 2048;
     hipLaunchKernelGGL(k_round_scan, dim3(wgrid), dim3(256), 0, s, Sl, state, nbrStart, nbrLow, nbr, waitOn, Unext, K, (int*)d_cnt, dfr.pend);
-    hipLaunchKernelGGL(k_round_emit, dim3(wgrid), dim3(256), 0, s, K, &d_cnt->nK, state, nbrStart, nbrCount, nbr, f, d_points, bbox,
+    hipLaunchKernelGGL(k_round_emit, dim3(wgrid), dim3(256), 0, s, K, &d_cnt->nK, state, g, cellRec, cellStart, by_bbox, reach, f, d_points, bbox,
                        radius, area, pairs, &d_cnt->nPairs, pairCap);
     SD_LAUNCH_CHECK();
     if (run_pairs(nullptr)) return -1;
@@ -1056,7 +1128,7 @@
   SD_CHECK(hipStreamSynchronize(s));
   if (stats) { stats[0] = totalPairs; stats[1] = totalExact; stats[2] = rounds; stats[3] = totalNbr;
                stats[4] = (int64_t)ns_pairs; stats[5] = n_pair_launches; stats[6] = (int64_t)ns_full; stats[7] = (int64_t)ns_pre;
-               stats[8] = totalSpill; stats[9] = totalDecided; stats[10] = totalUndecDeferred; }
+               stats[8] = totalSpill; stats[9] = totalDecided; stats[10] = totalUndecDeferred; stats[11] = totalSkipped; }
   if (verbose) {
     printf("NMS: %lld pair intersections (%lld on the exact-join path), %d greedy rounds, %lld neighbour entries\n",
            (long long)totalPairs, (long long)totalExact, rounds, (long long)totalNbr);
diff --git a/stardist_amd/csrc/nms_rounds.h b/stardist_amd/csrc/nms_rounds.h
--- a/stardist_amd/csrc/nms_rounds.h
+++ b/stardist_amd/csrc/nms_rounds.h
@@ -20,7 +20,7 @@
 __global__ void __launch_bounds__(256) k_sum_halves(const int* __restrict__ nLow, const int* __restrict__ nHigh, int N, unsigned long long* total) {
   __shared__ unsigned long long ws[4];
   unsigned long long v = 0;
-  for (int i = blockIdx.x * 256 + threadIdx.x; i < N; i += gridDim.x * 256) v += (unsigned long long)(nLow[i] + nHigh[i]);
+  for (int i = blockIdx.x * 256 + threadIdx.x; i < N; i += gridDim.x * 256) v += (unsigned long long)(nLow[i] + (nHigh ? nHigh[i] : 0));
   for (int o = 32; o; o >>= 1) v += __shfl_xor(v, o);
   if ((threadIdx.x & 63) == 0) ws[threadIdx.x >> 6] = v;
   __syncthreads();
@@ -121,6 +121,7 @@
   int* nbr; int* waitOn;
   long long total, slotTotal;
   bool slots;
+  bool lowOnly;
 };
 
 template <class LaunchNeighbours, class BeforeLists>
@@ -156,7 +157,7 @@
     if (!d_total) return -1;
     SD_CHECK(hipMemsetAsync(d_total, 0, sizeof(unsigned long long), s));
     launch(2, L);
-    hipLaunchKernelGGL(k_sum_halves, dim3(sd::div_up(N, 256) < 1024 ? sd::div_up(N, 256) : 1024), dim3(256), 0, s, L.low, L.count, N, d_total);
+    hipLaunchKernelGGL(k_sum_halves, dim3(sd::div_up(N, 256) < 1024 ? sd::div_up(N, 256) : 1024), dim3(256), 0, s, L.low, L.lowOnly ? (const int*)nullptr : L.count, N, d_total);
     SD_LAUNCH_CHECK();
     unsigned long long tot = 0;
     SD_CHECK(hipMemcpyAsync(&tot, d_total, sizeof(tot), hipMemcpyDeviceToHost, s));
diff --git a/stardist_amd/lib/_native.py b/stardist_amd/lib/_native.py
--- a/stardist_amd/lib/_native.py
+++ b/stardist_amd/lib/_native.py
@@ -27,6 +27,7 @@
     "sd_get_option": (_i, [ctypes.c_char_p]),
     "sd_nms2d_host": (_i, [_vp, _vp, _i, _i, _i, _i, _i, _f, _vp, _vp]),
     "sd_nms2d_device": (_i, [_vp, _vp, _i, _i, _i, _i, _i, _f, _vp, _vp, _vp]),
+    "sd_nms2d_build_device": (_i, [_vp, _vp, _i, _i, _vp, _vp, _vp, _vp, _vp, _vp, _vp]),
     "sd_nms2d_old_host": (_i, [_vp, _i, _i, _vp, _i, _i, _f, _i, _i, _i, _i, _vp]),
     "sd_nms2d_old_device": (_i, [_vp, _i, _i, _vp, _i, _i, _f, _i, _i, _i, _i, _vp, _vp]),
     "sd_clip_pairs_device": (_i, [_vp, _vp, _vp, _vp, _i, _i, _vp, _vp, _vp]),
diff --git a/stardist_amd/lib/stardist2d.py b/stardist_amd/lib/stardist2d.py
--- a/stardist_amd/lib/stardist2d.py
+++ b/stardist_amd/lib/stardist2d.py
@@ -147,6 +147,20 @@
     return out.cpu().numpy(), fl.cpu().numpy()
 
 
+def nms2d_build(dist, points):
+    import torch
+    N.require_device()
+    dev = torch.device("cuda")
+    d = torch.from_numpy(np.ascontiguousarray(dist, np.float32)).to(dev); p = torch.from_numpy(np.ascontiguousarray(points, np.float32)).to(dev)
+    n, R = d.shape
+    vx = torch.zeros((n, R), dtype=torch.int32, device=dev); vy = torch.zeros((n, R), dtype=torch.int32, device=dev)
+    bbox = torch.zeros((n, 4), dtype=torch.int32, device=dev); gstats = torch.zeros(5, dtype=torch.int32, device=dev)
+    radius = torch.zeros(n, dtype=torch.float32, device=dev); area = torch.zeros(n, dtype=torch.float32, device=dev)
+    N.dcall(d, "sd_nms2d_build_device", N.tptr(d), N.tptr(p), n, R, N.tptr(vx), N.tptr(vy), N.tptr(bbox), N.tptr(radius), N.tptr(area), N.tptr(gstats))
+    torch.cuda.synchronize()
+    return tuple(t.cpu().numpy() for t in (vx, vy, bbox, radius, area, gstats))
+
+
 def area_bounds_pairs(xa, ya, xb, yb):
     import torch
     N.require_device()
```

Result: faster. 318.7, median of 6 (+4.2%).
